# eflynn8/pharmacophore-diffusion

Hardware: AMD Instinct MI355X
Metric: denoising steps/sec (batch x T) at 256-atom pocket, 6 centers (higher is better)
Workload: dtype f32; 1 GPU; BASELINE config 2: 256-atom pocket, 6 centers, T=500 schedule, batch=32 per GPU, dev.yml network; batch_per_gpu=32, n_prot=256, n_pharm=6, T=500, parallelism=graphs sharded over 1 GPU(s), no data-path collective

## Files before the change

### include/pfdyn.h

```cpp
#ifndef PFDYN_H
#define PFDYN_H

#include <stdint.h>

#ifdef __cplusplus
extern "C" {
#endif

#define PF_ABI_VERSION 1

typedef struct pf_handle pf_handle;
typedef void* pf_stream;

typedef enum pf_status {
    PF_OK = 0,
    PF_ERR_ARG = -1,
    PF_ERR_HIP = -2,
    PF_ERR_STATE = -3,
    PF_ERR_WEIGHT = -4,
    PF_ERR_EXCHANGE = -5
} pf_status;

#define PF_NORM_MEAN 0
#define PF_NORM_VALUE 1
// ... 40 lines not shown
                        const float* dev_prot_x, const float* dev_prot_h,
                        int64_t n_pp, const int32_t* host_pp_src, const int32_t* host_pp_dst, pf_stream stream);

int pf_set_pocket_batch_host(pf_handle* h, int32_t B, const int32_t* host_prot_ptr, const int32_t* host_pharm_ptr,
                             const float* host_prot_x, const float* host_prot_h,
                             int64_t n_pp, const int32_t* host_pp_src, const int32_t* host_pp_dst, pf_stream stream);

int pf_set_pocket_groups(pf_handle* h, int32_t B, const int32_t* host_rep);

int pf_declare_onehot_features(pf_handle* h, int32_t is_onehot);

int64_t pf_build_pp_edges(pf_handle* h, int32_t B, const int32_t* host_prot_ptr, const float* dev_prot_x,
                          int32_t max_num_neighbors, int32_t* host_src, int32_t* host_dst, int64_t capacity,
                          pf_stream stream);

int pf_dynamics_forward(pf_handle* h, const float* dev_prot_x, const float* dev_pharm_x, const float* dev_pharm_h,
                        const float* dev_t , float* dev_eps_h , float* dev_eps_x ,
                        pf_stream stream);

int pf_sample_begin(pf_handle* h, const float* dev_init_pharm_com ,
                    const float* dev_noise0 , pf_stream stream);
int pf_denoise_step(pf_handle* h, const pf_step_coef* coef, const float* dev_noise ,
                    int32_t endpoint_param_coord, int32_t endpoint_param_feat, pf_stream stream);
int pf_sample_end(pf_handle* h, float feat_norm_constant, float* dev_x0 , float* dev_h0 ,
                  pf_stream stream);
int pf_sample_status(pf_handle* h, int32_t* n_timeouts);
int pf_sample_frame(pf_handle* h, float feat_norm_constant, float* dev_x , float* dev_h ,
                    pf_stream stream);
int pf_prepare_timesteps(pf_handle* h, const float* host_t, int32_t n, pf_stream stream);
int pf_sample(pf_handle* h, int32_t n_steps, const pf_step_coef* host_coef, const float* dev_noise,
              const float* dev_init_pharm_com, int32_t endpoint_param_coord, int32_t endpoint_param_feat,
              float feat_norm_constant, float* dev_x0, float* dev_h0, float* dev_traj_x, float* dev_traj_h,
              pf_stream stream);

int pf_param_count(pf_handle* h, int64_t* n_params, int32_t* n_tensors);
int pf_param_layout(pf_handle* h, int32_t index, const char** name, int64_t* offset, int64_t* numel);
int pf_train_forward(pf_handle* h, const float* dev_prot_x , const float* dev_pharm_x ,
                     const float* dev_pharm_h , const float* dev_t , float dropout_p, uint32_t seed,
                     float* dev_eps_h, float* dev_eps_x, pf_stream stream);
int pf_train_backward(pf_handle* h, const float* dev_g_eps_h , const float* dev_g_eps_x ,
                      float* dev_grad , pf_stream stream);
int pf_train_loss_forward(pf_handle* h, const float* dev_pharm_x0 , const float* dev_pharm_h0 ,
                          const int32_t* dev_t_int , const float* dev_eps_x , const float* dev_eps_h ,
                          const float* dev_alpha , const float* dev_sigma, int32_t n_timesteps, float feat_norm,
                          int32_t remove_com, int32_t weighted_loss, float dropout_p, uint32_t seed, float* dev_out ,
                          pf_stream stream);
int pf_train_loss_forward_ep(pf_handle* h, const float* dev_pharm_x0 , const float* dev_pharm_h0 ,
                             const int32_t* dev_t_int , const float* dev_eps_x , const float* dev_eps_h ,
                             const float* dev_alpha , const float* dev_sigma, int32_t n_timesteps, float feat_norm,
                             int32_t remove_com, int32_t weighted_loss, int32_t endpoint_param_coord, int32_t endpoint_param_feat,
                             float dropout_p, uint32_t seed, float* dev_out , pf_stream stream);
int pf_train_loss_backward(pf_handle* h, const float* dev_g_pos , const float* dev_g_feat ,
                           float* dev_grad , pf_stream stream);
int pf_train_loss_backward_out(pf_handle* h, const float* dev_g_out , float* dev_grad , pf_stream stream);
int pf_set_flat_params(pf_handle* h, const float* dev_flat , pf_stream stream);
int pf_get_flat_params(pf_handle* h, float* dev_flat , pf_stream stream);
int pf_adam_step(pf_handle* h, float* dev_params, const float* dev_grad, float* dev_exp_avg, float* dev_exp_avg_sq,
                 int64_t step, float lr, float beta1, float beta2, float eps, float weight_decay, pf_stream stream);
#define PF_TRAIN_F32 0
#define PF_TRAIN_BF16 1
int pf_train_set_precision(pf_handle* h, int32_t precision);
int pf_train_get_precision(pf_handle* h, int32_t* precision);
int pf_debug_set_dropout_masks(pf_handle* h, const float* dev_masks);
int pf_debug_dropout_mask(pf_handle* h, int32_t layer, int32_t which, float dropout_p, uint32_t seed,
                          float* dev_out , pf_stream stream);

int64_t pf_debug_get_edges(pf_handle* h, int32_t etype, int32_t* host_src, int32_t* host_dst, int64_t capacity,
                           pf_stream stream);
int pf_debug_conv_layer(pf_handle* h, int32_t layer, const float* dev_prot_x, const float* dev_pharm_x,
                        const float* dev_h_prot , const float* dev_v_prot ,
                        const float* dev_h_pharm, const float* dev_v_pharm,
                        float* dev_out_h_prot, float* dev_out_v_prot, float* dev_out_h_pharm, float* dev_out_v_pharm,
                        pf_stream stream);
#define PF_NUM_KERNEL_CLASSES 9
int pf_profile_enable(pf_handle* h, uint32_t kernel_mask);
int pf_profile_read(pf_handle* h, double* total_ms , int64_t* launches , pf_stream stream);
int pf_profile_read_train(pf_handle* h, double* total_ms , int64_t* launches , pf_stream stream);
int pf_debug_work(pf_handle* h, double* flops, double* bytes, int64_t* n_edges , double* executed_flops,
                  int64_t* executed_edges , pf_stream stream);
int pf_debug_counts(pf_handle* h, int64_t* out , pf_stream stream);
int pf_debug_kernel_family(pf_handle* h, int32_t layer, int32_t* rows_per_wave);
int pf_debug_ahead(pf_handle* h, int64_t* out , pf_stream stream);
int pf_debug_pa_check(pf_handle* h, int64_t* violations , pf_stream stream);
int pf_debug_xchg_timeouts(pf_handle* h, int32_t* n);
int pf_debug_xchg_fault(pf_handle* h, int32_t drop_word, int32_t poll_max);
int pf_debug_last_eps(pf_handle* h, float* dev_eps_h , float* dev_eps_x , pf_stream stream);
int pf_debug_l0_hoist(pf_handle* h, int32_t* rows_per_wave);
int pf_debug_chain(pf_handle* h, int32_t kind, int32_t layer, int32_t sub, int32_t n_rows, const float* dev_s_in,
                   const float* dev_v_in, float* dev_s_out, float* dev_v_out, pf_stream stream);

#ifdef __cplusplus
}
#endif
#endif
```

### pharmacophore-diffusion_amd/_lib.py

```python
import ctypes
import os

_HERE = os.path.dirname(os.path.abspath(__file__))
LIB_PATH = os.environ.get("PFDYN_LIB") or os.path.join(_HERE, "csrc", "libpfdyn.so")

PF_ABI_VERSION = 1
PF_NORM_MEAN, PF_NORM_VALUE, PF_NORM_GRAPH = 0, 1, 2


class PfConfig(ctypes.Structure):
    _fields_ = [
        ("abi_version", ctypes.c_int32), ("pharm_nf", ctypes.c_int32), ("rec_nf", ctypes.c_int32),
        ("vector_size", ctypes.c_int32), ("n_hidden_scalars", ctypes.c_int32), ("n_convs", ctypes.c_int32),
        ("n_message_gvps", ctypes.c_int32), ("n_update_gvps", ctypes.c_int32), ("n_noise_gvps", ctypes.c_int32),
        ("message_norm_mode", ctypes.c_int32), ("message_norm_value", ctypes.c_float),
        ("ff_k", ctypes.c_int32), ("pf_k", ctypes.c_int32),
        ("cutoff_pp", ctypes.c_float), ("cutoff_pf", ctypes.c_float), ("cutoff_fp", ctypes.c_float),
        ("cutoff_ff", ctypes.c_float), ("rbf_dmax", ctypes.c_float), ("rbf_dim", ctypes.c_int32),
    ]


class PfStepCoef(ctypes.Structure):
    _fields_ = [("t", ctypes.c_float), ("alpha_t_given_s", ctypes.c_float), ("var_terms", ctypes.c_float),
                ("sigma", ctypes.c_float), ("ep_zt", ctypes.c_float), ("ep_pred", ctypes.c_float)]


_P, _I32, _I64, _F = ctypes.c_void_p, ctypes.c_int32, ctypes.c_int64, ctypes.c_float
SYMBOLS = {
    "pf_version": (ctypes.c_char_p, []),
    "pf_last_error": (ctypes.c_char_p, [_P]),
    "pf_create": (ctypes.c_int, [ctypes.POINTER(PfConfig), ctypes.POINTER(_P)]),
    "pf_destroy": (None, [_P]),
    "pf_set_weight": (ctypes.c_int, [_P, ctypes.c_char_p, _P, _I32, ctypes.POINTER(_I64)]),
    "pf_commit_weights": (ctypes.c_int, [_P]),
    "pf_set_pocket_batch": (ctypes.c_int, [_P, _I32, _P, _P, _P, _P, _I64, _P, _P, _P]),
    "pf_set_pocket_batch_host": (ctypes.c_int, [_P, _I32, _P, _P, _P, _P, _I64, _P, _P, _P]),
    "pf_set_pocket_groups": (ctypes.c_int, [_P, _I32, _P]),
    "pf_declare_onehot_features": (ctypes.c_int, [_P, _I32]),
    "pf_build_pp_edges": (_I64, [_P, _I32, _P, _P, _I32, _P, _P, _I64, _P]),
    "pf_dynamics_forward": (ctypes.c_int, [_P, _P, _P, _P, _P, _P, _P, _P]),
    "pf_sample_begin": (ctypes.c_int, [_P, _P, _P, _P]),
    "pf_denoise_step": (ctypes.c_int, [_P, ctypes.POINTER(PfStepCoef), _P, _I32, _I32, _P]),
    "pf_sample_end": (ctypes.c_int, [_P, _F, _P, _P, _P]),
    "pf_sample_status": (ctypes.c_int, [_P, ctypes.POINTER(ctypes.c_int32)]),
    "pf_prepare_timesteps": (ctypes.c_int, [_P, _P, _I32, _P]),
    "pf_sample_frame": (ctypes.c_int, [_P, _F, _P, _P, _P]),
    "pf_sample": (ctypes.c_int, [_P, _I32, ctypes.POINTER(PfStepCoef), _P, _P, _I32, _I32, _F, _P, _P, _P, _P, _P]),
    "pf_param_count": (ctypes.c_int, [_P, ctypes.POINTER(_I64), ctypes.POINTER(_I32)]),
    "pf_param_layout": (ctypes.c_int, [_P, _I32, ctypes.POINTER(ctypes.c_char_p), ctypes.POINTER(_I64), ctypes.POINTER(_I64)]),
    "pf_train_forward": (ctypes.c_int, [_P, _P, _P, _P, _P, _F, ctypes.c_uint32, _P, _P, _P]),
    "pf_train_backward": (ctypes.c_int, [_P, _P, _P, _P, _P]),
    "pf_train_loss_forward": (ctypes.c_int, [_P, _P, _P, _P, _P, _P, _P, _P, ctypes.c_int32, ctypes.c_float, ctypes.c_int32,
                                             ctypes.c_int32, ctypes.c_float, ctypes.c_uint32, _P, _P]),
    "pf_train_loss_forward_ep": (ctypes.c_int, [_P, _P, _P, _P, _P, _P, _P, _P, ctypes.c_int32, ctypes.c_float, ctypes.c_int32,
                                                ctypes.c_int32, ctypes.c_int32, ctypes.c_int32, ctypes.c_float, ctypes.c_uint32, _P, _P]),
    "pf_train_loss_backward": (ctypes.c_int, [_P, _P, _P, _P, _P]),
    "pf_train_loss_backward_out": (ctypes.c_int, [_P, _P, _P, _P]),
    "pf_set_flat_params": (ctypes.c_int, [_P, _P, _P]),
    "pf_get_flat_params": (ctypes.c_int, [_P, _P, _P]),
    "pf_adam_step": (ctypes.c_int, [_P, _P, _P, _P, _P, _I64, _F, _F, _F, _F, _F, _P]),
    "pf_train_set_precision": (ctypes.c_int, [_P, _I32]),
    "pf_train_get_precision": (ctypes.c_int, [_P, ctypes.POINTER(_I32)]),
    "pf_debug_set_dropout_masks": (ctypes.c_int, [_P, _P]),
    "pf_debug_dropout_mask": (ctypes.c_int, [_P, _I32, _I32, _F, ctypes.c_uint32, _P, _P]),
    "pf_debug_get_edges": (_I64, [_P, _I32, _P, _P, _I64, _P]),
    "pf_debug_conv_layer": (ctypes.c_int, [_P, _I32] + [_P] * 11),
    "pf_profile_enable": (ctypes.c_int, [_P, ctypes.c_uint32]),
    "pf_profile_read": (ctypes.c_int, [_P, ctypes.POINTER(ctypes.c_double), ctypes.POINTER(_I64), _P]),
    "pf_profile_read_train": (ctypes.c_int, [_P, ctypes.POINTER(ctypes.c_double), ctypes.POINTER(_I64), _P]),
    "pf_debug_work": (ctypes.c_int, [_P, ctypes.POINTER(ctypes.c_double), ctypes.POINTER(ctypes.c_double),
                                     ctypes.POINTER(_I64), ctypes.POINTER(ctypes.c_double), ctypes.POINTER(_I64), _P]),
    "pf_debug_counts": (ctypes.c_int, [_P, ctypes.POINTER(_I64), _P]),
    "pf_debug_kernel_family": (ctypes.c_int, [_P, ctypes.c_int32, ctypes.POINTER(ctypes.c_int32)]),
    "pf_debug_last_eps": (ctypes.c_int, [_P, _P, _P, _P]),
    "pf_debug_xchg_timeouts": (ctypes.c_int, [_P, ctypes.POINTER(ctypes.c_int32)]),
    "pf_debug_xchg_fault": (ctypes.c_int, [_P, _I32, _I32]),
    "pf_debug_ahead": (ctypes.c_int, [_P, ctypes.POINTER(_I64), _P]),
    "pf_debug_pa_check": (ctypes.c_int, [_P, ctypes.POINTER(_I64), _P]),
    "pf_debug_l0_hoist": (ctypes.c_int, [_P, ctypes.POINTER(ctypes.c_int32)]),
    "pf_debug_chain": (ctypes.c_int, [_P, _I32, _I32, _I32, _I32, _P, _P, _P, _P, _P]),
}

_lib = None


def load():
    global _lib
    if _lib is not None:
        return _lib
    if not os.path.exists(LIB_PATH):
        raise ImportError(
            f"{LIB_PATH} is missing: the HIP extension has not been built "
            "(run `python -c 'import __graft_entry__ as g; g.build()'` or `make -C pharmacophore-diffusion_amd/csrc`). "
            "There is no CPU fallback.")
    lib = ctypes.CDLL(LIB_PATH)
    for name, (res, args) in SYMBOLS.items():
        fn = getattr(lib, name)
        fn.restype = res
        fn.argtypes = args
    _lib = lib
    return lib


class PfError(RuntimeError):
    pass


def check(lib, handle, rc, what):
    if rc < 0:
        msg = lib.pf_last_error(handle)
        raise PfError(f"{what} failed ({rc}): {msg.decode() if msg else ''}")
    return rc
```

### pharmacophore-diffusion_amd/csrc/pf_device.h

```cpp
#pragma once
#include <stdint.h>

#define PF_S 128
#define PF_V 16
#define PF_R 16
#define PF_MAXF 64
#define PF_MAXK 16
#define PF_MAX_GVPS 8

enum { ET_FF = 0, ET_PF = 1, ET_FP = 2, ET_PP = 3 };

#if defined(__HIP_DEVICE_COMPILE__)
#define PF_AS1 __attribute__((address_space(1)))
#else
#define PF_AS1
#endif
typedef const float PF_AS1* pf_gcf;

struct GvpW {
    pf_gcf a_wh;
    pf_gcf a_wu;
    pf_gcf a_main;
    pf_gcf a_main_c;
    pf_gcf a_gate_c;
// ... 103 lines not shown
    const int* esrc;
    const int* edst;
    const float4* xn;
    const float* h;
    const float* v;
    float* msg_s;
    float* msg_v;
    const GvpW* w;
    const float* pre;
    int n_gvps;
    float rbf_mu[PF_R];
    float rbf_inv_sigma;
    float* sv_z; float* sv_g; float* sv_v; size_t sv_stride;
    int bf16;
    pf_gcf rg[4];
    const int* reg; int nreg, regB, ngroups4, ngroups8;
    pf_gcf rgs[4]; int rgs_stride;
    const float* zs;
    const float* ptab;
    int ptab_gstride;
    const int* ptype;
    const int* eorig;
    const int* l0_gid;
    const float* l0c;
    int ngroups_sel;
    const int* need; int need_stamp;
    int pa_abs;
    pf_gcf n16[4]; int n16_stride[4];
    int uni_base[3], uni_s01, uni_s2g, uni_pa_groups;
    int ptab16_off[4];
    const float* pcen; int pcen_nf;
    const float* x0_static;
    const int* pa_skip;
    int* cnt_snap;
    int* pa_gstamp; int pa_serial;
};

#define L0H_WR 0
#define L0H_WSH 2048
#define L0H_B 4224
#define L0H_WH0 4352
#define L0H_WU 4384
#define L0H_BG 4672
#define L0H_WHT 4736
#define L0H_WHT_PF 21120
#define L0H_B_PF 37504
#define L0H_SIZE (37504 + 128)
#define L0C_WHT_FF 0
#define L0C_B_FF 16384
#define L0C_WHT_FP 16512
#define L0C_B_FP 32896
#define L0C_SIZE (32896 + 128)
#define L0_NTAB 4
struct L0HoistParams {
    const float* src;
    float* l0c;
    const int* esrc; const int* edst; const float4* xn; int Epp;
    float rbf_mu0, rbf_mu_step, rbf_inv_sigma;
    float* zs;
    const float* enc_w; const float* enc_b; const float* enc_lw; const float* enc_lb;
    int rec_nf, nt;
    const float* t_dev;
    float t_host[64];
    float* ptab;
    const float* prot_h0; int Np; int* ptype; int* flag;
};

struct NodeW {
    pf_gcf ln1_w; pf_gcf ln1_b;
    pf_gcf ln2_w; pf_gcf ln2_b;
    const GvpW PF_AS1* upd;
};

struct UnitParams {
    const float* s_in; const float* v_in; float* s_out; float* v_out;
    int n, kind, n_gvps, pharm_nf;
    const float* stream;
    int skip_gvps;
    const float* ln_w; const float* ln_b;
    float* sv_z; float* sv_g; float* sv_v; size_t sv_stride;
    int n16_stride;
};

struct NodeParams {
    const NodeTile* tiles;
    int ntiles;
    const int* in_start;
    const int* in_cnt;
    int N;
    int pp_slot;
    const int* row_ids;
    const int* dyn_cnt;
    const float* msg_s;
    const float* msg_v;
    int zero_row;
    const float* h_in; const float* v_in;
    float* h_out; float* v_out;
    const int* gid;
    const float* gnorm;
    int B;
    int norm_mode; float norm_value;
    NodeW w[2];
    int n_upd;
    uint32_t drop_thr; float drop_scale; uint32_t seed; int layer;
    const float* mask_override;
    int xcd_n;
    int st_n0, st_n;
    int grp;
    int grp_pa;
    pf_gcf rg_upd[2];
    pf_gcf rgs_upd[2]; int rgs_stride[2];
    float* sv_z; float* sv_g; float* sv_v; size_t sv_stride;
};

struct ZeroList {
    void* p[8];
    unsigned long long nbytes[8];
    int cnt;
};
struct FusedParams {
    const int* in_start; const int* in_cnt; int N, pp_slot;
    const float* msg_s; const float* msg_v; int zero_row, grp, grp_pa;
    const int* gid; const float* gnorm; int B, norm_mode; float norm_value;
    pf_gcf ln1_w[2], ln1_b[2], ln2_w[2], ln2_b[2];
    int n_upd;
    pf_gcf chain[4]; int chain_stride[4];
    pf_gcf upd_pharm; int upd_pharm_stride;
    const float* htab; int htab_gstride;
    const int* ptype;
    float* h_out; float* v_out;
    const int* pharm_ptr; int Np, n_edge_items;
    int xcd_split, nff_cap, npf_cap;
    int uni_ff_base, uni_pf_base, uni_strides, uni_groups;
    const int4* rec;
    const float* hcen;
};

struct TailParams {
    const int* in_start; const int* in_cnt; int N;
    const float* msg_s; const float* msg_v; int zero_row, grp;
    const float* h_in; const float* v_in;
    const int* gid; const float* gnorm; int B, norm_mode; float norm_value;
    pf_gcf ln1_w, ln1_b, ln2_w, ln2_b;
    int n_upd, n_head;
    pf_gcf chain; int chain_stride;
    int pharm_nf;
    float* eps_h; float* eps_x;
};

struct HeadParams {
    const NodeTile* tiles;
    int ntiles;
    int node_base;
    const float* h; const float* v;
    const GvpW* gvps;
    int n_gvps;
    const float* a_out;
    const float* b_out;
    int pharm_nf;
    float* eps_h;
    float* eps_x;
    unsigned int* xchg;
    int xchg_fault;
    unsigned int* xchg2;
};
#define PF_XCHG_STRIDE 20
#define PF_XCHG_EMPTY 0xffffffffu
#ifdef __HIPCC__
__device__ __forceinline__ unsigned int pf_xchg_word(const float v) {
    const unsigned int b = __float_as_uint(v);
    return b == PF_XCHG_EMPTY ? 0x7fc00000u : b;
}
#endif

struct CenHoistParams {
    int on, Nf, nf;
    float t_next;
    const float* pharm_h;
    const float* noise;
    float a_ts, var, sigma, ep_zt, ep_pred; int ep_feat;
    const float* enc_w; const float* enc_b; const float* enc_lw; const float* enc_lb;
    const float* blk;
    float* cen_h; float* cen_p;
    unsigned int* xchg2;
};

struct EncodeParams {
    int Np, Nf;
    const float* prot_h0;
    const float* pharm_h;
    const float* t;
    float t_scalar;
    const int* gid;
    int rec_nf, pharm_nf;
    const float* w[2]; const float* b[2]; const float* ln_w[2]; const float* ln_b[2];
    float* h_out;
};

struct BuildParams {
    int B, Np_tot;
    const int* prot_ptr; const int* pharm_ptr;
    const float4* xn;
    const int* reg;
    int* dyn_cnt;
    int* act_ids;
    const int* reg_act;
    int* esrc; int* edst;
    int* eorig;
    int* in_start; int* in_cnt; int N;
    int ff_k, pf_k;
    float r2_ff, r2_pf;
    float* gnorm;
    const int* pp_cnt;
    const int* pa_static;
    const int* rep_base;
    int* need; int need_stamp;
    const int* pfq_cnt;
    int norm_mode;
// ... 86 lines not shown
```

### pharmacophore-diffusion_amd/csrc/pf_host.cpp

```cpp
#include <hip/hip_runtime.h>

#include <algorithm>
#include <cmath>
#include <cstdio>
#include <cstdlib>
#include <cstring>
#include <ctime>
#include <map>
#include <string>
#include <unordered_map>
#include <climits>
#include <vector>

#include "../../include/pfdyn.h"
#include "pf_device.h"
#include "pf_train.h"

#define L0_PTAB_SLOTS 2048

extern "C" {
void pfk_edge_msg(const EdgeParams* p, int layer0, hipStream_t s);
void pfk_edge_msg_coop(const EdgeParams* p, int layer0, hipStream_t s);
void pfk_edge_msg_coop2(const EdgeParams* p, int layer0, hipStream_t s);
void pfk_node_update_coop(const NodeParams* p, int layer0, hipStream_t s);
void pfk_node_head_coop(const NodeParams* p, const HeadParams* hp, int layer0, hipStream_t s);
void pfk_noise_head_coop(const HeadParams* p, hipStream_t s);
void pfk_node_update(const NodeParams* p, int layer0, hipStream_t s);
void pfk_noise_head(const HeadParams* p, hipStream_t s);
void pfk_rg_edge(const EdgeParams* p, const EncodeParams* enc, int layer0, int rg, int split, int rgp, hipStream_t s);
void pfk_l0_hoist(const L0HoistParams* p, int what, hipStream_t s);
void pfk_rg_node(const NodeParams* p, const HeadParams* hp, const EncodeParams* enc, int layer0, int rg, int split, hipStream_t s);
void pfk_rg_unit(const UnitParams* p, hipStream_t s);
void pfk_rg_node_hs_build(const NodeParams* p, const HeadParams* hp, const StepParams* sp, const BuildParams* bp, int* xstat, int poll_sleep,
                          int avoid, int poll_max, const CenHoistParams* cp, const EdgeParams* es, const EncodeParams* ees, int spec_groups,
                          hipStream_t s);
void pfk_n16_edge(const EdgeParams* p, const EncodeParams* enc, int layer0, hipStream_t s);
void pfk_pa_spec(const EdgeParams* es, const EncodeParams* ees, int groups, int after, int k, int frac, int* word, hipStream_t s);
void pfk_pa_check(const int* dyn_cnt, const int* cnt_snap, const int* reg, const int* pa_same, const int* gstamp, int serial, int B,
                  unsigned long long* out, hipStream_t s);
void pfk_n16_unit(const UnitParams* p, hipStream_t s);
void pfk_n16_fused(const EdgeParams* p, const FusedParams* f, const EncodeParams* enc, hipStream_t s);
void pfk_n16_tail(const TailParams* t, const StepParams* sp, const BuildParams* bp, hipStream_t s);
void pfk_rg_tail(const NodeParams* p, const HeadParams* hp, const StepParams* sp, const BuildParams* bp, hipStream_t s);
void pfk_encode(const EncodeParams* p, hipStream_t s);
void pfk_encode_build(const EncodeParams* e, const BuildParams* b, hipStream_t s);
void pfk_encode_build_pre(const EncodeParams* e, const BuildParams* b, const PreParams* pp, hipStream_t s);
void pfk_build_edges(const BuildParams* p, hipStream_t s);
void pfk_load_coords(const float* src, float4* xn, int n, const int* gid, const float* shift, float sign, hipStream_t s);
void pfk_load_noise0(const float* nz, float4* xn, float* hf, int n, int nf, hipStream_t s);
void pfk_copy(const float* src, float* dst, size_t n, hipStream_t s);
void pfk_zero_multi(const ZeroList* z, hipStream_t s);
void pfk_copy2(const float* a, float* da, size_t na, const float* b, float* db, size_t nb, hipStream_t s);
void pfk_verify_copies(const float* x0, const float* h0, const int* gid, const int* prot_ptr, const int* rep_base, int Np, int rec_nf,
                       int* flag, hipStream_t s);
void pfk_scale_copy(const float* src, float* dst, size_t n, float sc, hipStream_t s);
void pfk_segment_mean(const float4* xn, const int* ptr, int base, int B, float* out, hipStream_t s);
void pfk_step_update(const StepParams* p, hipStream_t s);
void pfk_step_build(const StepParams* sp, const BuildParams* bp, int fast, hipStream_t s);
void pfk_export_coords(const float4* xn, int base, int n, const int* gid, const float* add, const float* sub,
                       float* out, hipStream_t s);
void pfk_bwd_head(const BwdHeadParams* p, int nblocks, hipStream_t s);
void pfk_bwd_node(const BwdNodeParams* p, int nblocks, hipStream_t s);
void pfk_bwd_edge_level(const BwdEdgeLevelParams* p, int nblocks, hipStream_t s);
void pfk_fix_apply(long long* A, float* G, size_t n, const float* fix, hipStream_t s);
void pfk_fix_apply_rows(const NodeTile* tiles, int ntiles, const int* dyn_cnt, const int* row_ids, long long* A_h, float* G_h,
                        long long* A_v, float* G_v, const float* fix, hipStream_t s);
void pfk_fix_scale(const float* g_h, int n_h, const float* g_x, int n_x, float* fix, hipStream_t s);
void pfk_bwd_encode(const BwdEncodeParams* p, int nblocks, hipStream_t s);
void pfk_enc_group(const float* G_h, const int* prot_ptr, const int* ptype, int B, int rec_nf, float* Gg, hipStream_t s);
void pfk_fix_enc_group(long long* A_h, float* G_h, const float* fix, const int* prot_ptr, const int* ptype, int B, int rec_nf, float* Gg,
                       int Np, int Nf, const int* onehot_flag, hipStream_t s);
void pfk_train_reduce(const ReduceParams* p, hipStream_t s);
void pfk_gather_weights(const float* flat, const int* map, size_t n, float* packed, hipStream_t s);
void pfk_n16_split_words(const float* flat, const int4* tab, size_t n, float* packed, hipStream_t s);
void pfk_pack_gvp(const float* W, const GvpT* g, int n_gvps, float* out_b, float* out_f, const ScaleArgs* sa, hipStream_t s);
void pfk_loss_prepare(const LossParams* p, hipStream_t s);
void pfk_loss_eval(const LossParams* p, int ep_coord, int ep_feat, hipStream_t s);
void pfk_scale_loss(float* gx, int nx, const float* a, const float* a2, float* gh, int nh, const float* b, const float* b2, hipStream_t s);
void pfk_compact_node_rows(const NodeTile* tiles, int ntiles, const int* dyn_cnt, const int* row_ids, int N, int* list, int cap, int* ucnt,
                           hipStream_t s);
void pfk_compact_rows(const EdgeTile* tiles, const int* et_tile0, int n_et, const int* dyn_cnt, int* rlist, int* ccnt, hipStream_t s);
void pfk_adam(float* p, const float* g, float* m, float* v, size_t n, float lr, float b1, float b2, float eps, float wd,
              float bc1, float bc2_sqrt, float* mirror, hipStream_t s);
void pfk_drop_masks(const TrainCommon* c, uint32_t stream, int n_elems, float* out, hipStream_t s);
void pfk_pp_radius(const float4* xn, const int* prot_ptr, int B, float r2, int maxn, int* deg, const int* row_off,
                   int* src, int* dst, int pass, hipStream_t s);
void pfk_wide_encode(const WideEncParams* p, hipStream_t s);
void pfk_wide_edge(const WideEdgeParams* p, hipStream_t s);
void pfk_wide_node(const WideNodeParams* p, hipStream_t s);
}

namespace {

static std::string g_create_error;

struct RawTensor {
    std::vector<int64_t> shape;
    std::vector<float> data;
};

static const char* kEtKey[4] = {"pharm_ff_pharm", "prot_pf_pharm", "pharm_fp_prot", "prot_pp_prot"};
static const char* kNtKey[2] = {"prot", "pharm"};

inline int rho(int r, int hl) { return (r & 3) + 8 * (r >> 2) + 4 * hl; }

static void linspace_f32(float start, float end, int steps, float* out) {
    const float step = (end - start) / (float)(steps - 1);
    const int half = steps / 2;
    for (int i = 0; i < steps; ++i) out[i] = i < half ? start + step * (float)i : end - step * (float)(steps - i - 1);
}

}

struct LaunchPolicy {
    static constexpr int kCUs = 256, kSIMDs = 4 * kCUs;
    int n16_mask = 7;
    int tail_graphs_max = 256;
    int xcd_split = 1;
// ... 63 lines not shown
    std::vector<GvpW> h_gvp;
    int msg_base(int layer, int et) const { return ((layer * 4 + et) * cfg.n_message_gvps); }
    int upd_base(int layer, int nt) const { return n_msg_tot + (layer * 2 + nt) * cfg.n_update_gvps; }
    int head_base() const { return n_msg_tot + n_upd_tot; }
    int n_msg_tot = 0, n_upd_tot = 0;
    size_t enc_w[2]{}, enc_b[2]{}, enc_lw[2]{}, enc_lb[2]{};
    std::vector<size_t> ln_off;
    size_t out_a = 0, out_b = 0;
    size_t enc_a = 0, enc_bf = 0;
    bool use_pre = true;

    bool have_batch = false;
    int B = 0, Np = 0, Nf = 0, N = 0;
    int64_t Epp = 0, Ecap = 0;
    std::vector<int> h_prot_ptr, h_pharm_ptr;
    std::vector<int> h_reg;
    std::vector<int> h_cap;
    int n_edge_tiles = 0, n_node_tiles = 0, n_head_tiles = 0;
    int zero_row = 0;
    int n_edge_tiles_last = 0, n_node_tiles_last = 0;
    bool prune = true;
    int n_edge_tiles_act = 0, n_node_tiles_act = 0;
    EdgeTile* d_edge_tiles_act = nullptr;
    NodeTile* d_node_tiles_act = nullptr;
    int *d_act_ids = nullptr, *d_reg_act = nullptr;
    void* d_ws = nullptr;
    size_t ws_capacity = 0;
    void* stage[2] = {nullptr, nullptr};
    size_t stage_cap[2] = {0, 0};
    hipEvent_t stage_ev[2] = {nullptr, nullptr};
    int stage_next = 0;
    void* d_tab[2] = {nullptr, nullptr};
    size_t tab_cap[2] = {0, 0};
    hipEvent_t tab_guard[2] = {nullptr, nullptr}, tab_up[2] = {nullptr, nullptr};
    bool tab_guard_set[2] = {false, false};
    int tab_next = 0;
    hipStream_t s_copy = nullptr;
    hipStream_t s_side = nullptr;
    int l0_state = 0;
    int* l0flag_host = nullptr;
    hipEvent_t l0flag_ev = nullptr;
    size_t tws_capacity = 0;
    int *d_prot_ptr = nullptr, *d_pharm_ptr = nullptr, *d_gid = nullptr, *d_reg = nullptr, *d_dyn_cnt = nullptr,
        *d_esrc = nullptr, *d_edst = nullptr, *d_in_start = nullptr, *d_in_cnt = nullptr, *d_pp_cnt = nullptr;
    EdgeTile* d_edge_tiles = nullptr;
    NodeTile* d_node_tiles = nullptr;
    NodeTile* d_head_tiles = nullptr;
    float4* d_xn = nullptr;
    float *d_prot_x0 = nullptr, *d_prot_h0 = nullptr, *d_pharm_h = nullptr, *d_t = nullptr, *d_h[2] = {nullptr, nullptr},
          *d_v[2] = {nullptr, nullptr}, *d_msg_s = nullptr, *d_msg_v = nullptr, *d_eps_h = nullptr, *d_eps_x = nullptr,
          *d_com_init = nullptr, *d_com_tmp = nullptr, *d_gnorm = nullptr, *d_pre = nullptr;
    int* d_pfq_cnt = nullptr;
    std::vector<int> pending_rep;
    bool share_ok = false;
    int share_check = 1;
    int* d_reg_share = nullptr;
    int* d_pa_static = nullptr;
    int* d_rep_base = nullptr;
    int* d_need = nullptr;
    int need_stamp = 0, edges_stamp = 0;
    long share_rows = 0;
    std::vector<int> h_share_start, h_share_cnt;
    bool share_disable = false;
    bool train_rg_node = true;
    bool train_rg_edge = true;
    bool train_rg_head = true;
    float *t_hsv_z = nullptr, *t_hsv_g = nullptr, *t_hsv_v = nullptr;
    bool t_head_saved = false;
    unsigned int* d_xchg = nullptr;
    int* d_xstat = nullptr;
    int* xstat_host = nullptr;
    int xstat_ack = 0;
    int xchg_fault = 0, xchg_poll_max = 0;
    size_t n16_l0h[4] = {0, 0, 0, 0}, n16_l0h_stride[4] = {0, 0, 0, 0};
    size_t l0c_off = 0;
    bool cen_hoist = true;
    float *d_cen_h = nullptr, *d_cen_p = nullptr, *d_snap[2] = {nullptr, nullptr};
    unsigned int* d_xchg2 = nullptr;
    int snap_cur = -1;
    std::vector<float> t_plan; size_t plan_pos = 0;
    bool cen_valid = false; float cen_t = 0.f; uint64_t cen_wver = 0;
    bool last_cen = false;
    bool pa_spec = true;
    bool spec_valid = false; float spec_t = 0.f; uint64_t spec_wver = 0;
    int step_id = 2;
    int *d_pa_stamp = nullptr, *d_pa_same = nullptr;
    bool e0_saved = false; EdgeParams e0{}; EncodeParams ep0{}; int e0_groups = 0;
    int last_spec = 0;
    int* d_pa_cnt = nullptr;
    int pa_spec_split = 0;
    bool pa_check = false;
    int pa_serial = 0, spec_serial = 0;
    int* d_pa_gstamp = nullptr;
    unsigned long long* d_pa_chk = nullptr;
    bool no_fixed_shapes = false;
    ScaleArgs pend_scale{}; bool has_pend_scale = false;
    bool no_fix_fuse = false;
    bool train_bf16 = false;
    bool train_node_save = true;
    std::vector<float*> t_nsv_z, t_nsv_g, t_nsv_v;
    std::vector<char> t_node_saved;
    std::vector<int> t_grp;
    bool sampling = false;
    int max_np = 0, max_nf = 0;
    bool edges_built = false;
    bool edges_share = false;
    std::vector<size_t> rg_msg, rg_upd;
    std::vector<size_t> rgs_msg, rgs_upd, rgs_upd_stride;
    size_t rgs_msg_stride = 0;
    std::vector<size_t> n16_msg, n16_upd;
    size_t n16_msg_stride = 0, n16_upd_stride = 0;
    size_t n16_begin = 0;
    bool n16_stale = false;
    bool split_record = false;
    std::vector<int4> split_pending, split_tab;
    int4* d_split_tab = nullptr; size_t n_split_tab = 0;
    size_t n16_l0[4] = {0, 0, 0, 0}, n16_l0_stride[4] = {0, 0, 0, 0};
    size_t n16_fused[2] = {0, 0}, n16_fused_stride[2] = {0, 0};
    size_t n16_tail = 0, n16_tail_stride = 0;
    bool tail_done = false;
    int last_tail = 0;
    float *d_msg_s2 = nullptr, *d_msg_v2 = nullptr;
    std::vector<int> last_family;
    int last_hoist = 0;
    bool l0_hoist = true;
    size_t l0h_off = 0;
    uint64_t w_version = 1, zs_version = 0, ptab_version = 0;
    bool l0_onehot = false;
    bool coords_custom = false;
    bool zs_batch_coords = false;
    float* d_l0c = nullptr;
    float* d_ptab = nullptr;
    std::unordered_map<uint32_t, int> ptab_slot;
    int *d_eorig = nullptr, *d_ptype = nullptr, *d_l0flag = nullptr;
    int4* d_rec = nullptr; bool rec_valid = false;
    float *d_zs = nullptr, *d_ptab_pg = nullptr;
    bool enc_on_the_fly = true;
    bool step_build_fast = true;
    bool rg_compact = true;
    bool fuse_head = true;
    void init_tuning() {
        if (const char* e = getenv("PFDYN_NO_PRE")) use_pre = atoi(e) == 0;
        if (const char* e = getenv("PFDYN_NO_FUSE_HEAD")) fuse_head = atoi(e) == 0;
        if (const char* e = getenv("PFDYN_NO_PRUNE")) prune = atoi(e) == 0;
        if (const char* e = getenv("PFDYN_NO_ENC_FLY")) enc_on_the_fly = atoi(e) == 0;
        if (const char* e = getenv("PFDYN_NO_COMPACT")) rg_compact = atoi(e) == 0;
        if (const char* e = getenv("PFDYN_NO_FAST_BUILD")) step_build_fast = atoi(e) == 0;
        if (const char* e = getenv("PFDYN_NO_L0_HOIST")) l0_hoist = atoi(e) == 0;
        if (const char* e = getenv("PFDYN_NO_CENTER_HOIST")) cen_hoist = atoi(e) == 0;
        if (const char* e = getenv("PFDYN_NO_PA_SPEC")) pa_spec = atoi(e) == 0;
        if (const char* e = getenv("PFDYN_PA_SPEC_SPLIT")) pa_spec_split = !strcmp(e, "mid") ? -1 : (!strcmp(e, "step") ? -2 : std::max(atoi(e), 0));
        if (const char* e = getenv("PFDYN_PA_CHECK")) pa_check = atoi(e) != 0;
        if (const char* e = getenv("PFDYN_NO_POCKET_SHARE")) share_disable = atoi(e) != 0;
        if (const char* e = getenv("PFDYN_TRAIN_TILE_NODE")) train_rg_node = atoi(e) == 0;
        if (const char* e = getenv("PFDYN_TRAIN_TILE_EDGE")) train_rg_edge = atoi(e) == 0;
        if (const char* e = getenv("PFDYN_TRAIN_TILE_HEAD")) train_rg_head = atoi(e) == 0;
        if (const char* e = getenv("PFDYN_TRAIN_NODE_RECOMPUTE")) train_node_save = atoi(e) == 0;
        if (const char* e = getenv("PFDYN_TRAIN_BF16")) train_bf16 = atoi(e) != 0;
        if (const char* e = getenv("PFDYN_NO_FIX_FUSE")) no_fix_fuse = atoi(e) != 0;
        if (const char* e = getenv("PFDYN_NO_FIXED_SHAPES")) no_fixed_shapes = atoi(e) != 0;
        pol.from_env();
    }

    float* d_flat = nullptr;
    size_t nparams = 0;
    std::vector<std::pair<std::string, std::pair<size_t, size_t>>> flat_layout;
    GvpT* d_gvpt = nullptr;
    std::vector<int> h_map;
    int* d_map = nullptr;
    size_t n_packed = 0;
    void* d_tws = nullptr;
    std::vector<float*> t_H, t_V, t_msg_s, t_msg_v;
    std::vector<float*> t_sv_z, t_sv_g, t_sv_v;
    float *t_gs_buf = nullptr, *t_gv_buf = nullptr;
    int et_tile0[5] = {0, 0, 0, 0, 0};
    int et_tile0_act[5] = {0, 0, 0, 0, 0};
    float *t_G_h[2] = {nullptr, nullptr}, *t_G_v[2] = {nullptr, nullptr}, *t_gagg_s = nullptr, *t_gagg_v = nullptr,
          *t_gpart = nullptr, *t_geps_h = nullptr, *t_geps_x = nullptr;
    long long *t_A_h = nullptr, *t_A_v = nullptr;
    float* d_lpart = nullptr;
    void* d_tA = nullptr;
    size_t tA_capacity = 0;
    bool tA_dirty = false;
    int enc_begin = 0, enc_n = 0;
    float* t_gpart_enc = nullptr;
    TensorSeg* d_tseg = nullptr; int n_tseg = 0;
    int n_gvpt = 0;
    float* d_wpack = nullptr;
    uint64_t wpack_version = ~0ull;
    float *t_lx0c = nullptr, *t_lag = nullptr, *t_lsg = nullptr, *t_lcom2 = nullptr, *t_lgx = nullptr, *t_lgh = nullptr, *t_lout = nullptr;
    bool t_have_loss = false;
    float* t_Gg = nullptr;
    int* t_ulist = nullptr;
    int t_ucap = 0;
    size_t t_clist_cap = 0, t_ulist_cap = 0;
    hipEvent_t cmp_ev[3] = {nullptr, nullptr, nullptr};
    int *t_clist = nullptr, *t_ccnt = nullptr;
    float* t_fix = nullptr;
    int t_nblk = 0;
    const float* t_mask_override = nullptr;
    bool t_have_fwd = false;
    bool t_ws_ready = false;
    TrainCommon t_common{};
    mutable std::unordered_map<std::string, size_t> flat_index;
    mutable bool flat_index_ok = false;
    size_t flat_offset(const std::string& name) const {
        if (!flat_index_ok) {
            flat_index.clear();
            for (const auto& kv : flat_layout) flat_index.emplace(kv.first, kv.second.first);
            flat_index_ok = true;
        }
        const auto it = flat_index.find(name);
        return it == flat_index.end() ? (size_t)-1 : it->second;
    }
    std::vector<int> edge_fx;

    enum { K_ENCODE = 0, K_BUILD, K_EDGE, K_NODE, K_HEAD, K_STEP, K_EDGE_COOP, K_NODE_COOP, K_EDGE_LAST,
           K_BWD_HEAD, K_BWD_NODE, K_BWD_EDGE_LEVEL, K_BWD_REST, K_NUM };
    unsigned prof_mask = 0;
    std::vector<std::pair<hipEvent_t, hipEvent_t>> prof_ev[K_NUM];
    size_t prof_used[K_NUM] = {};
};

namespace {

#define PF_FAIL(h, code, ...)                                   \
    do {                                                        \
        char _b[512];                                           \
        snprintf(_b, sizeof(_b), __VA_ARGS__);                  \
        (h)->err = _b;                                          \
        return (code);                                          \
    } while (0)

// ... 766 lines not shown
        e.x0_static = h->d_prot_x0;
        if (dc.spec_have && pa_ahead_ok(h, e, shared)) { e.pa_skip = h->d_pa_same; h->last_spec = 1; }
    }
    if (l == 0 && dc.cen_have && h->n16_l0h[ET_FF] != 0) {
        for (int et : {(int)ET_FF, (int)ET_FP}) { e.n16[et] = h->d_w + h->n16_l0h[et]; e.n16_stride[et] = (int)h->n16_l0h_stride[et]; }
        e.pcen = h->d_cen_p; e.pcen_nf = h->Nf; h->last_cen = true;
    }
    e.ngroups_sel = region_groups(h, shared, 0, e.nreg, 16);
    int stride[3], cap[3], grp[3] = {0, 0, 0};
    bool uni = l == 0 && h->pol.fused_uni && !shared && e.reg == h->d_reg && e.nreg == 4 * h->B && h->B <= 64 && !e.pa_abs && !e.need &&
               uniform_regions(h, 3, stride, cap);
    for (int et = 0; et < 3 && uni; ++et) { grp[et] = (cap[et] + 15) / 16; uni = grp[et] > 0 && grp[et] < 8; }
    if (uni) {
        for (int et = 0; et < 3; ++et) e.uni_base[et] = h->h_reg[(size_t)et * h->B];
        e.uni_s01 = stride[0] | (stride[1] << 16);
        e.uni_s2g = stride[2] | (grp[0] << 16) | (grp[1] << 19) | (grp[2] << 22) | ((h->B - 1) << 25);
        e.uni_pa_groups = region_groups(h, shared, 3 * h->B, 4 * h->B, 16);
    }
    dc.rg = 4;
    if (l == 0 && e.x0_static && pa_ahead_ok(h, e, shared)) {
        e.cnt_snap = h->d_pa_cnt;
        h->e0 = e; h->ep0 = dc.ep; h->e0_saved = true;
        h->e0_groups = region_groups(h, shared, 3 * h->B, 4 * h->B, 16);
    }
}
static void edge_launch(DynCall& dc, int l) {
    pf_handle* h = dc.h; hipStream_t s = dc.s; const pf_config& c = h->cfg; const bool train = dc.train;
    const bool last = dc.last = (l == c.n_convs - 1), pruned = dc.pruned = (l == prune_layer(h));
    EdgeParams& e = dc.e; int &rg = dc.rg, &rgp = dc.rgp;
    e = edge_params_base(h, l, last, pruned);
    e.h = train ? h->t_H[l] : h->d_h[dc.cur]; e.v = train ? h->t_V[l] : h->d_v[dc.cur];
    e.msg_s = train ? h->t_msg_s[l] : h->d_msg_s; e.msg_v = train ? h->t_msg_v[l] : h->d_msg_v;
    if (dc.fuse_l0node && l == 1) { e.msg_s = h->d_msg_s2; e.msg_v = h->d_msg_v2; }
    e.pre = (l == 0 && dc.pre_ready) ? h->d_pre : nullptr;
    if (train) { e.sv_z = h->t_sv_z[l]; e.sv_g = h->t_sv_g[l]; e.sv_v = h->t_sv_v[l]; e.sv_stride = (size_t)std::max<int64_t>(h->Ecap, 1); }
    const bool shared = dc.shared = dc.share && pruned && l == 0;
    if ((last || pruned) && h->rg_compact && (last ? 2 : 4) * h->B <= 1024) {
        e.reg = shared ? h->d_reg_share : h->d_reg; e.regB = h->B; e.nreg = (last ? 2 : 4) * h->B; e.pa_abs = shared ? 1 : 0;
        if (shared) { e.need = h->d_need; e.need_stamp = h->edges_stamp; }
        e.ngroups4 = region_groups(h, shared, 0, e.nreg, 4); e.ngroups8 = region_groups(h, shared, 0, e.nreg, 8);
    }
    if (train && h->train_bf16) e.bf16 = 1;
    rg = train ? ((h->train_rg_edge && h->train_rg_node && !h->train_bf16) ? h->pol.rg_mode(e.ntiles) : 0)
               : h->pol.rg_mode(shared ? (int)((h->share_rows + 31) / 32) : e.ntiles);
    rgp = 0;
    if (dc.hoist && l == 0 && rg) {
        e.zs = h->d_zs; e.ptab = dc.l0_ptab; e.ptab_gstride = dc.l0_gstride; e.ptype = h->d_ptype; e.eorig = h->d_eorig; e.l0_gid = h->d_gid; e.l0c = h->d_l0c;
        rgp = rg;
        if (e.nreg > 0 && pruned) {
            rg = shared ? ((h->share_rows >= h->pol.rg2_rows_min || (long)e.ntiles * 32 >= h->pol.rg2_rows_min_hoist) ? 2 : 1)
                        : ((long)e.ntiles * 32 >= h->pol.rg2_rows_min_hoist ? 2 : 1);
            const int rgp_pol = shared ? rg : ((long)e.ntiles * 32 >= h->pol.rg2p_rows_min ? 2 : 1);
            if (h->pol.l0_rga) rg = h->pol.l0_rga;
            rgp = h->pol.l0_rgp ? h->pol.l0_rgp : std::max(rg, rgp_pol);
            if (rg == 2) rgp = 2;
            e.ngroups_sel = region_groups(h, shared, 0, 3 * h->B, 4 * rg) + region_groups(h, shared, 3 * h->B, e.nreg, 4 * rgp);
        }
        h->last_hoist = 4 * rgp;
    }
    const bool n16e = !train && rg && dc.n16_batch && (l > 0 ? (h->pol.n16_mask & 1) != 0 : dc.n16_l0);
    if (n16e) edge_n16_form(dc, l);
    h->last_family.resize(c.n_convs);
    h->last_family[l] = rg ? 4 * rg : ((!train && e.ntiles <= ((last || pruned) ? std::max(h->pol.coop_edge_max, h->pol.coop2_edge_max) : std::max(h->pol.coop_edge_max, h->pol.coop2_dense_max))) ? 128 : 32);
    for (int et = 0; et < 4; ++et) { e.rgs[et] = h->d_w + h->rgs_msg[(size_t)l * 4 + et]; e.rgs_stride = (int)h->rgs_msg_stride; }
    const int esplit = (rg == 1 && e.ntiles * 8 <= h->pol.rg_split_max && !e.zs) ? 1 : 0;
    const int pc = edge_prof_class(last, c.n_convs);
    if (n16e && dc.fuse_l0node && l == 1) {
        FusedParams& fz = dc.fz;
        fz.chain[ET_FF] = h->d_w + h->n16_fused[0]; fz.chain_stride[ET_FF] = (int)h->n16_fused_stride[0];
        fz.chain[ET_PF] = h->d_w + h->n16_fused[1]; fz.chain_stride[ET_PF] = (int)h->n16_fused_stride[1];
        fz.upd_pharm = h->d_w + h->n16_upd[(size_t)0 * 2 + 1]; fz.upd_pharm_stride = (int)h->n16_upd_stride;
        fz.htab = dc.l0_ptab + (size_t)3 * c.rec_nf * PF_S; fz.htab_gstride = dc.l0_gstride; fz.ptype = h->d_ptype; fz.hcen = h->last_cen ? h->d_cen_h : nullptr;
        fz.h_out = h->d_h[dc.cur]; fz.v_out = h->d_v[dc.cur];
        fz.pharm_ptr = h->d_pharm_ptr; fz.Np = h->Np; fz.n_edge_items = e.ngroups_sel;
        fz.nff_cap = region_groups(h, shared, 0, std::min(h->B, e.nreg), 16); fz.npf_cap = region_groups(h, shared, h->B, e.nreg, 16);
        fz.xcd_split = ((h->pol.xcd_split & 1) && 2 * h->B <= 64 && h->max_nf <= 16) ? 1 : 0;
        int stride[2], cap[2];
        bool uni = fz.xcd_split && h->pol.fused_uni && e.reg == h->d_reg && e.nreg == 2 * h->B && uniform_regions(h, 2, stride, cap);
        for (int et = 0; et < 2 && uni; ++et) uni = cap[et] > 0 && (cap[et] + 15) / 16 < 256;
        if (uni) {
            fz.uni_ff_base = h->h_reg[0]; fz.uni_pf_base = h->h_reg[(size_t)h->B];
            fz.uni_strides = stride[0] | (stride[1] << 16); fz.uni_groups = ((cap[0] + 15) / 16) | (((cap[1] + 15) / 16) << 8);
        }
        h->last_family[l] = 17;
        { ProfScope ps(h, pf_handle::K_EDGE_LAST, s); pfk_n16_fused(&e, &fz, &dc.ep, s); }
    }
    else if (n16e) {
        if (l == 0 && e.pa_skip && h->d_pa_gstamp && h->d_pa_chk)
            pfk_pa_check(h->d_dyn_cnt, h->d_pa_cnt, e.reg, e.pa_skip, h->d_pa_gstamp, h->spec_serial, h->B, h->d_pa_chk, s);
        ProfScope ps(h, pc, s); pfk_n16_edge(&e, &dc.ep, l == 0, s);
    }
    else if (rg) { ProfScope ps(h, pc, s); pfk_rg_edge(&e, dc.enc_fly ? &dc.ep : nullptr, l == 0, rg, esplit, rgp, s); }
    else if (e.ntiles <= h->pol.coop_edge_max && !train) { ProfScope ps(h, pc, s); pfk_edge_msg_coop(&e, l == 0, s); }
    else if (e.ntiles <= ((last || pruned) ? h->pol.coop2_edge_max : h->pol.coop2_dense_max) && !train) { ProfScope ps(h, pc, s); pfk_edge_msg_coop2(&e, l == 0, s); }
    else { ProfScope ps(h, pf_handle::K_EDGE, s); pfk_edge_msg(&e, l == 0, s); }
}
static void fused_take_node(DynCall& dc, const NodeParams& n) {
    pf_handle* h = dc.h; FusedParams& fz = dc.fz;
    fz.in_start = n.in_start; fz.in_cnt = n.in_cnt; fz.N = n.N; fz.pp_slot = n.pp_slot;
    fz.rec = (h->rec_valid && h->d_rec && n.pp_slot == 2 && !dc.shared) ? h->d_rec : nullptr;
    fz.msg_s = n.msg_s; fz.msg_v = n.msg_v; fz.zero_row = n.zero_row; fz.grp = n.grp; fz.grp_pa = n.grp_pa;
    fz.gid = n.gid; fz.gnorm = n.gnorm; fz.B = n.B; fz.norm_mode = n.norm_mode; fz.norm_value = n.norm_value; fz.n_upd = n.n_upd;
    for (int nt = 0; nt < 2; ++nt) { fz.ln1_w[nt] = n.w[nt].ln1_w; fz.ln1_b[nt] = n.w[nt].ln1_b; fz.ln2_w[nt] = n.w[nt].ln2_w; fz.ln2_b[nt] = n.w[nt].ln2_b; }
}
static void node_save_levels(pf_handle* h, int l, NodeParams& n) {
    n.sv_z = h->t_nsv_z[l]; n.sv_g = h->t_nsv_g[l]; n.sv_v = h->t_nsv_v[l]; n.sv_stride = (size_t)2 * h->N;
    h->t_node_saved[l] = 1;
}
static void tail_launch(DynCall& dc, const NodeParams& n, int form) {
    pf_handle* h = dc.h; hipStream_t s = dc.s; const pf_config& c = h->cfg;
    const HeadParams hp = head_params(h, dc.eps_h, dc.eps_x); TailParams tp{};
    if (form == 16) {
        tp.in_start = n.in_start; tp.in_cnt = n.in_cnt; tp.N = n.N; tp.h_in = n.h_in; tp.v_in = n.v_in;
        tp.msg_s = n.msg_s; tp.msg_v = n.msg_v; tp.zero_row = n.zero_row; tp.grp = n.grp;
        tp.gid = n.gid; tp.gnorm = n.gnorm; tp.B = n.B; tp.norm_mode = n.norm_mode; tp.norm_value = n.norm_value;
        tp.ln1_w = n.w[1].ln1_w; tp.ln1_b = n.w[1].ln1_b; tp.ln2_w = n.w[1].ln2_w; tp.ln2_b = n.w[1].ln2_b;
        tp.n_upd = n.n_upd; tp.n_head = c.n_noise_gvps; tp.chain = h->d_w + h->n16_tail; tp.chain_stride = (int)h->n16_tail_stride;
        tp.pharm_nf = c.pharm_nf; tp.eps_h = dc.eps_h; tp.eps_x = dc.eps_x;
    }
    const bool sn = share_next(h);
    const BuildParams bpn = build_params(h, sn);
    { ProfScope ps(h, pf_handle::K_HEAD, s); if (form == 16) pfk_n16_tail(&tp, dc.step, &bpn, s); else pfk_rg_tail(&n, &hp, dc.step, &bpn, s); }
    build_done(h, sn);
    h->tail_done = true; h->last_tail = form; dc.head_done = true;
}
static float cen_hoist_plan(DynCall& dc) {
    pf_handle* h = dc.h;
    if (!(h->cen_hoist && dc.t_scalar && !h->t_plan.empty() && h->last_hoist == 16 && h->l0c_off != 0 && h->n16_l0h[ET_FF] != 0 &&
          h->snap_cur >= 0 && dc.step->h_snap_out != nullptr && h->d_xchg2 && dc.fuse_l0node)) return NAN;
    return planned_next_t(h, *dc.t_scalar, &h->plan_pos);
}
static void cen_hoist_params(DynCall& dc, float t_next, CenHoistParams& cp, HeadParams& hp) {
    pf_handle* h = dc.h; const StepParams* step = dc.step;
    cp.on = 1; cp.Nf = h->Nf; cp.nf = h->cfg.pharm_nf; cp.t_next = t_next; cp.pharm_h = h->d_snap[h->snap_cur]; cp.noise = step->noise;
    cp.a_ts = step->a_ts; cp.var = step->var; cp.sigma = step->sigma; cp.ep_zt = step->ep_zt; cp.ep_pred = step->ep_pred; cp.ep_feat = step->ep_feat;
    cp.enc_w = h->d_w + h->enc_w[1]; cp.enc_b = h->d_w + h->enc_b[1]; cp.enc_lw = h->d_w + h->enc_lw[1]; cp.enc_lb = h->d_w + h->enc_lb[1];
    cp.blk = h->d_w + h->l0c_off; cp.cen_h = h->d_cen_h; cp.cen_p = h->d_cen_p; cp.xchg2 = hp.xchg2 = h->d_xchg2;
    h->cen_valid = true; h->cen_t = t_next; h->cen_wver = h->w_version;
}
static int pa_ahead_plan(DynCall& dc, EdgeParams& es, EncodeParams& ees) {
    pf_handle* h = dc.h; const pf_config& c = h->cfg;
    if (!(h->e0_saved && h->pa_spec && !h->t_plan.empty() && dc.t_scalar && h->d_pa_stamp && !share_next(h))) return 0;
    float tn = planned_next_t(h, *dc.t_scalar, nullptr);
    if (tn != tn) return 0;
    l0_prepare_t(h, &tn, 1, dc.s);
    uint32_t bits; memcpy(&bits, &tn, 4);
    es = h->e0; es.pa_skip = nullptr; es.pcen = nullptr;
    es.ptab = h->d_ptab + (size_t)h->ptab_slot[bits] * L0_NTAB * c.rec_nf * PF_S;
    for (int et = 0; et < 4; ++et) { es.n16[et] = h->d_w + h->n16_l0[et]; es.n16_stride[et] = (int)h->n16_l0_stride[et]; }
    ees = h->ep0; ees.t_scalar = tn;
    h->spec_valid = true; h->spec_t = tn; h->spec_wver = h->w_version;
    es.pa_serial = h->spec_serial = ++h->pa_serial; es.pa_gstamp = h->d_pa_gstamp;
    return h->e0_groups;
}
static void merged_step_launch(DynCall& dc, const NodeParams& n, HeadParams& hp) {
    pf_handle* h = dc.h; hipStream_t s = dc.s; const pf_config& c = h->cfg;
    hp.xchg = h->d_xchg; hp.xchg_fault = h->xchg_fault;
    CenHoistParams cp{}; EdgeParams es{}; EncodeParams ees{};
    const float t_next = cen_hoist_plan(dc);
    const int spec_groups = pa_ahead_plan(dc, es, ees);
    if (t_next == t_next) cen_hoist_params(dc, t_next, cp, hp);
    const bool sn = share_next(h);
    BuildParams bpn = build_params(h, sn);
    const bool with_rec = h->d_rec && !sn && c.ff_k == 0 && bpn.act_ids && !bpn.pa_static && h->last_hoist == 16 && dc.fuse_l0node;
    if (with_rec) { bpn.rec = h->d_rec; bpn.ptype = h->d_ptype; }
    const bool split = spec_groups > 0 && h->pa_spec_split != 0;
    if (split) {
        const int frac = h->pa_spec_split == -1 ? 128 : (h->pa_spec_split == -2 ? (int)((((uint32_t)h->pa_serial * 2654435761u) >> 16) & 255) + 1 : 0);
        pfk_pa_spec(&es, &ees, spec_groups, 0, std::max(h->pa_spec_split, 0), frac, h->d_pa_cnt + h->B, s);
    }
    { ProfScope ps(h, pf_handle::K_HEAD, s); pfk_rg_node_hs_build(&n, &hp, dc.step, &bpn, h->d_xstat, h->pol.xchg_sleep, h->pol.hsb_avoid, h->xchg_poll_max, &cp, &es, &ees, split ? 0 : spec_groups, s); }
    if (split) pfk_pa_spec(&es, &ees, spec_groups, 1, 0, 0, h->d_pa_cnt + h->B, s);
    build_done(h, sn, with_rec);
    h->tail_done = true; h->last_tail = 2;
}
static void node_launch(DynCall& dc, int l) {
    pf_handle* h = dc.h; hipStream_t s = dc.s; const pf_config& c = h->cfg; const bool train = dc.train;
    NodeParams n = node_params_base(h, l, dc.last, dc.pruned);
    if (dc.shared) n.pp_slot = 3;
    n.msg_s = dc.e.msg_s; n.msg_v = dc.e.msg_v; n.h_in = dc.e.h; n.v_in = dc.e.v;
    n.h_out = train ? h->t_H[l + 1] : h->d_h[dc.cur ^ 1]; n.v_out = train ? h->t_V[l + 1] : h->d_v[dc.cur ^ 1];
    if (train) { n.drop_thr = h->t_common.drop_thr; n.drop_scale = h->t_common.drop_scale; n.seed = h->t_common.seed; n.layer = l; n.mask_override = h->t_common.mask_override; }
    n.grp = dc.rg ? 4 * dc.rg : 32; n.grp_pa = dc.rgp ? 4 * dc.rgp : n.grp;
    if (train) { h->t_grp.resize(c.n_convs); h->t_grp[l] = n.grp; h->t_node_saved.resize(c.n_convs); h->t_node_saved[l] = 0; }
    for (int nt = 0; nt < 2; ++nt) { n.rgs_upd[nt] = h->d_w + h->rgs_upd[(size_t)l * 2 + nt]; n.rgs_stride[nt] = (int)h->rgs_upd_stride[(size_t)l * 2 + nt]; }
    const EncodeParams* enc = dc.enc_fly ? &dc.ep : nullptr;
    if (dc.fuse_l0node && l == 0) fused_take_node(dc, n);
    else if (dc.rg) {
        const int rgn = (long)n.ntiles * 32 >= h->pol.rg2_rows_min_node ? 2 : 1;
        const bool fuse = dc.last && !train && h->fuse_head && h->n_head_tiles == n.ntiles;
        const int nsplit = (!train && rgn == 1 && n.ntiles * 8 <= (fuse ? h->pol.rg_split_max_head : h->pol.rg_split_max_node)) ? 1 : 0;
        const bool tail = fuse && dc.step != nullptr && l > 0 && (h->pol.n16_mask & 8) && h->B <= h->pol.tail_graphs_max && dc.enc_fly && step_build_fast_ok(h);
        if (tail) tail_launch(dc, n, (h->pol.tail_form == 16 && h->n16_tail != 0) ? 16 : 4);
        else if (fuse) {
            if (nsplit && h->pol.node_xcds > 0 && n.ntiles * 8 <= 32 * h->pol.node_xcds) n.xcd_n = h->pol.node_xcds;
            if (nsplit && l > 0 && h->pol.node_static) { n.st_n0 = h->Np; n.st_n = h->Nf; }
            HeadParams hp = head_params(h, dc.eps_h, dc.eps_x);
            const bool hsb = n.st_n > 0 && dc.step != nullptr && h->pol.hs_build && dc.enc_fly && step_build_fast_ok(h) &&
                             h->B <= 256 && !(h->prof_mask & (1u << pf_handle::K_STEP)) && h->d_xchg && h->d_xstat;
            if (hsb) merged_step_launch(dc, n, hp);
            else { ProfScope ps(h, pf_handle::K_HEAD, s); pfk_rg_node(&n, &hp, enc, l == 0, rgn, nsplit, s); }
            dc.head_done = true;
        } else {
            if (train && h->train_node_save) node_save_levels(h, l, n);
            ProfScope ps(h, pf_handle::K_NODE_COOP, s); pfk_rg_node(&n, nullptr, enc, l == 0, rgn, nsplit, s);
        }
    }
    else if (dc.last && !train && h->fuse_head && n.ntiles <= h->pol.coop_node_max && h->n_head_tiles == n.ntiles) {
        const HeadParams hp = head_params(h, dc.eps_h, dc.eps_x);
        { ProfScope ps(h, pf_handle::K_HEAD, s); pfk_node_head_coop(&n, &hp, l == 0, s); }
        dc.head_done = true;
    }
    else if (train && h->train_rg_node && h->pol.rg_mode(n.ntiles) > 0) {
        n.grp = 32; n.grp_pa = 32;
        if (h->train_node_save) node_save_levels(h, l, n);
        ProfScope ps(h, pf_handle::K_NODE_COOP, s); pfk_rg_node(&n, nullptr, nullptr, l == 0, h->pol.rg_mode(n.ntiles), 0, s);
    }
    else if (n.ntiles <= h->pol.coop_node_max && !train) { ProfScope ps(h, pf_handle::K_NODE_COOP, s); pfk_node_update_coop(&n, l == 0, s); }
    else { ProfScope ps(h, pf_handle::K_NODE, s); pfk_node_update(&n, l == 0, s); }
}
static void head_launch(DynCall& dc) {
    pf_handle* h = dc.h; hipStream_t s = dc.s; const pf_config& c = h->cfg; const bool train = dc.train;
    HeadParams hp = head_params(h, dc.eps_h, dc.eps_x);
    hp.h = train ? h->t_H[c.n_convs] : h->d_h[dc.cur]; hp.v = train ? h->t_V[c.n_convs] : h->d_v[dc.cur];
    if (train) h->t_head_saved = false;
    if (!dc.head_done && train && h->train_rg_head && !h->rg_msg.empty() && h->Nf > 0) {
        UnitParams up{};
        up.s_in = hp.h + (size_t)h->Np * PF_S; up.v_in = hp.v + (size_t)h->Np * 48; up.s_out = dc.eps_h; up.v_out = dc.eps_x;
        up.n = h->Nf; up.kind = 3; up.n_gvps = c.n_noise_gvps; up.pharm_nf = c.pharm_nf;
        up.stream = h->d_w + h->rg_upd[(size_t)(c.n_convs - 1) * 2 + 1]; up.skip_gvps = c.n_update_gvps;
        up.sv_z = h->t_hsv_z; up.sv_g = h->t_hsv_g; up.sv_v = h->t_hsv_v; up.sv_stride = (size_t)h->Nf;
        { ProfScope ps(h, pf_handle::K_HEAD, s); pfk_rg_unit(&up, s); }
        h->t_head_saved = true; dc.head_done = true;
    }
    if (!dc.head_done) { ProfScope ps(h, pf_handle::K_HEAD, s); if (hp.ntiles <= h->pol.coop_node_max) pfk_noise_head_coop(&hp, s); else pfk_noise_head(&hp, s); }
}
static int run_dynamics(pf_handle* h, float* eps_h, float* eps_x, hipStream_t s, const float* t_scalar = nullptr, bool train = false, const StepParams* step = nullptr) {
    if (h->wide && !train) return run_dynamics_wide(h, eps_h, eps_x, s, t_scalar);
    const pf_config& c = h->cfg;
    h->tail_done = false; h->last_tail = 0;
    DynCall dc{};
    dc.h = h; dc.s = s; dc.eps_h = eps_h; dc.eps_x = eps_x; dc.t_scalar = t_scalar; dc.train = train; dc.step = step;
    dc.cen_have = !train && h->cen_valid && h->edges_built && t_scalar != nullptr && *t_scalar == h->cen_t && h->cen_wver == h->w_version;
    h->cen_valid = false; h->last_cen = false;
    dc.spec_have = !train && h->spec_valid && h->edges_built && t_scalar != nullptr && *t_scalar == h->spec_t && h->spec_wver == h->w_version;
    h->spec_valid = false; h->last_spec = 0; h->e0_saved = false;
    if (!train) n16_refresh(h, s);
    dc.ep = encode_params(h, t_scalar, train ? h->t_H[0] : h->d_h[0]);
    if (const int rc = dyn_prologue(dc)) return rc;
    dyn_hoist_prepare(dc);
    h->last_hoist = 0;
    dc.fuse_l0node = !train && dc.n16_batch && (long)h->n_edge_tiles_act * 32 <= h->pol.n16_fuse_rows_max && (h->pol.n16_mask & 4) && (h->pol.n16_mask & 1) && dc.hoist && c.n_convs == 2 && prune_layer(h) == 0 && c.pf_k > 0 &&
                     c.n_update_gvps >= 1 && h->rg_compact && 2 * h->B <= 1024 && h->d_msg_s2 != nullptr && h->n16_fused[0] != 0;
    for (int l = 0; l < c.n_convs; ++l, dc.cur ^= 1) { edge_launch(dc, l); node_launch(dc, l); }
    head_launch(dc);
    h->edges_built = h->tail_done;
    hipError_t e = hipGetLastError();
    if (e != hipSuccess) PF_FAIL(h, PF_ERR_HIP, "kernel launch failed: %s", hipGetErrorString(e));
    return PF_OK;
}

struct ZeroBatch {
    ZeroList z{};
    hipStream_t s;
    explicit ZeroBatch(hipStream_t st) : s(st) {}
    void add(void* p, size_t nbytes) {
        if (!p || nbytes == 0) return;
        if (z.cnt == 8) flush();
        z.p[z.cnt] = p; z.nbytes[z.cnt] = nbytes; ++z.cnt;
    }
    void flush() { pfk_zero_multi(&z, s); z.cnt = 0; }
};

static int check_ready(pf_handle* h, bool need_batch) {
    if (!h) return PF_ERR_ARG;
    if (!h->committed) PF_FAIL(h, PF_ERR_STATE, "weights not committed (pf_commit_weights)");
    if (need_batch && !h->have_batch) PF_FAIL(h, PF_ERR_STATE, "no pocket batch set (pf_set_pocket_batch)");
    return PF_OK;
}

}

extern "C" {

const char* pf_version(void) { return "libpfdyn 0.1 (gfx950, fp32 MFMA)"; }

const char* pf_last_error(const pf_handle* h) { return h ? h->err.c_str() : g_create_error.c_str(); }

int pf_create(const pf_config* cfg, pf_handle** out) {
    if (!cfg || !out) { g_create_error = "null argument"; return PF_ERR_ARG; }
    *out = nullptr;
    auto bad = [&](const char* m) { g_create_error = m; return PF_ERR_ARG; };
    if (cfg->abi_version != PF_ABI_VERSION) return bad("abi_version mismatch");
    if (cfg->vector_size != 16 && cfg->vector_size != PFW_MAXV) return bad("vector_size must be 16 or 32");
    if (cfg->n_hidden_scalars < 64 || cfg->n_hidden_scalars > PFW_MAXS || cfg->n_hidden_scalars % 32)
        return bad("n_hidden_scalars must be a multiple of 32 in 64..256");
    if (cfg->rbf_dim != PF_R) return bad("rbf_dim must be 16");
    if (cfg->pharm_nf < 1 || cfg->pharm_nf > 16 || cfg->rec_nf < 1) return bad("pharm_nf must be in 1..16, rec_nf >= 1");
    if (cfg->n_convs < 1 || cfg->n_message_gvps < 1 || cfg->n_message_gvps > PF_MAX_GVPS || cfg->n_update_gvps < 1 ||
        cfg->n_update_gvps > PF_MAX_GVPS || cfg->n_noise_gvps < 1 || cfg->n_noise_gvps > PF_MAX_GVPS)
        return bad("layer counts out of range");
    if (cfg->ff_k < 0 || cfg->ff_k > PF_MAXK || cfg->pf_k < 0 || cfg->pf_k > PF_MAXK) return bad("ff_k / pf_k must be in 0..16");
    if (cfg->message_norm_mode < 0 || cfg->message_norm_mode > 2) return bad("bad message_norm_mode");
    if (cfg->message_norm_mode == PF_NORM_VALUE && !(cfg->message_norm_value > 0)) return bad("message_norm_value must be > 0");
    int ndev = 0;
    if (hipGetDeviceCount(&ndev) != hipSuccess || ndev == 0) {
        g_create_error = "no HIP device available (libpfdyn has no CPU fallback)";
        return PF_ERR_HIP;
    }
    pf_handle* h = new pf_handle();
    h->cfg = *cfg;
    h->init_tuning();
    h->spec = cfg->n_hidden_scalars == PF_S && cfg->vector_size == PF_V;
    const char* wv = getenv("PFDYN_WIDE");
    h->wide = !h->spec || (wv && atoi(wv) != 0);
    if (h->wide) {
        h->l0_hoist = h->cen_hoist = h->pa_spec = false;
        h->pol.hs_build = 0; h->pol.n16_mask = 0;
    }
    *out = h;
    return PF_OK;
}

void pf_destroy(pf_handle* h) {
// ... 152 lines not shown
                for (int k = 0; k < 17; ++k) blk[L0H_WH0 + k] = wh[(size_t)0 * 17 + k];
                for (int k = 0; k < 17 * 16; ++k) blk[L0H_WU + k] = wu[k];
                for (int k = 0; k < 16; ++k) blk[L0H_BG + k] = h->raw[g.prefix + "scalar_to_vector_gates.bias"].data[k];
                const GvpSpec gp = msg_spec(c, 0, ET_PF, 0);
                const std::vector<float>& Wp = h->raw[gp.prefix + "to_feats_out.0.weight"].data;
                for (int f = 0; f < PF_S; ++f) {
                    for (int k = 0; k < PF_S; ++k) blk[L0H_WHT_PF + (size_t)k * PF_S + f] = Wp[(size_t)f * Kin + k];
                    blk[L0H_B_PF + f] = h->raw[gp.prefix + "to_feats_out.0.bias"].data[f];
                }
            }
            h->l0h_off = push(h->h_w, blk);
            h->l0c_off = 0;
            if (g.vi == 17 && g.so == PF_S && g.si == PF_S + PF_R && g.vo == 16) {
                std::vector<float> cb(L0C_SIZE, 0.f);
                const int Kin = g.si + 17;
                for (int k2 = 0; k2 < 2; ++k2) {
                    const GvpSpec gc = msg_spec(c, 0, k2 == 0 ? ET_FF : ET_FP, 0);
                    const std::vector<float>& Wc = h->raw[gc.prefix + "to_feats_out.0.weight"].data;
                    const std::vector<float>& bc = h->raw[gc.prefix + "to_feats_out.0.bias"].data;
                    const size_t wo = k2 == 0 ? L0C_WHT_FF : L0C_WHT_FP, bo = k2 == 0 ? L0C_B_FF : L0C_B_FP;
                    for (int f = 0; f < PF_S; ++f) {
                        for (int k = 0; k < PF_S; ++k) cb[wo + (size_t)k * PF_S + f] = Wc[(size_t)f * Kin + k];
                        cb[bo + f] = bc[f];
                    }
                }
                h->l0c_off = push(h->h_w, cb);
            }
        }
        if (h->spec) {
            h->rg_msg.assign((size_t)c.n_convs * 4, 0);
            h->rg_upd.assign((size_t)c.n_convs * 2, 0);
            std::vector<float> st;
            auto flush = [&]() { const size_t off = push(h->h_w, st); st.clear(); return off; };
            auto chain = [&](auto spec_of, int n, int half = -1) {
                GvpSpec prev;
                for (int j = 0; j < n; ++j) {
                    const GvpSpec g = spec_of(j);
                    pack_gvp_rg(h, g, j ? &prev : nullptr, st, half);
                    prev = g;
                }
                pack_flush_rg(h, prev, st);
            };
            for (int l = 0; l < c.n_convs; ++l)
                for (int et = 0; et < 4; ++et) {
                    chain([&](int j) { return msg_spec(c, l, et, j); }, c.n_message_gvps);
                    h->rg_msg[(size_t)l * 4 + et] = flush();
                }
            for (int l = 0; l < c.n_convs; ++l)
                for (int nt = 0; nt < 2; ++nt) {
                    if (l == c.n_convs - 1 && nt == 1) continue;
                    chain([&](int j) { return upd_spec(c, l, nt, j); }, c.n_update_gvps);
                    h->rg_upd[(size_t)l * 2 + nt] = flush();
                }
            chain([&](int j) { return upd_spec(c, c.n_convs - 1, 1, j); }, c.n_update_gvps);
            chain([&](int k) { return head_spec(c, k); }, c.n_noise_gvps);
            pack_out_rg(h, st);
            st.resize(st.size() + (size_t)RG_TAIL_PAD * 256, 0.f);
            h->rg_upd[(size_t)(c.n_convs - 1) * 2 + 1] = flush();
            h->rgs_msg.assign((size_t)c.n_convs * 4, 0);
            h->rgs_upd.assign((size_t)c.n_convs * 2, 0);
            h->rgs_upd_stride.assign((size_t)c.n_convs * 2, 0);
            for (int l = 0; l < c.n_convs; ++l)
                for (int et = 0; et < 4; ++et) {
                    for (int half = 0; half < 2; ++half) {
                        chain([&](int j) { return msg_spec(c, l, et, j); }, c.n_message_gvps, half);
                        if (half == 0) h->rgs_msg_stride = st.size();
                    }
                    h->rgs_msg[(size_t)l * 4 + et] = flush();
                }
            for (int l = 0; l < c.n_convs; ++l)
                for (int nt = 0; nt < 2; ++nt) {
                    const bool tail = l == c.n_convs - 1 && nt == 1;
                    for (int half = 0; half < 2; ++half) {
                        chain([&](int j) { return upd_spec(c, l, nt, j); }, c.n_update_gvps, half);
                        if (tail) {
                            chain([&](int k) { return head_spec(c, k); }, c.n_noise_gvps, half);
                            pack_out_rg(h, st);
                        }
                        if (half == 0) h->rgs_upd_stride[(size_t)l * 2 + nt] = st.size();
                    }
                    if (!tail) h->rgs_upd[(size_t)l * 2 + nt] = flush();
                }
            st.resize(st.size() + (size_t)RG_TAIL_PAD * 256, 0.f);
            h->rgs_upd[(size_t)(c.n_convs - 1) * 2 + 1] = flush();
        }
        h->n16_begin = h->spec ? h->h_w.size() : 0;
        if (h->spec && c.n_message_gvps >= 2 && c.n_update_gvps >= 1) {
            h->n16_msg.assign((size_t)c.n_convs * 4, 0);
            h->n16_upd.assign((size_t)c.n_convs * 2, 0);
            std::vector<float> st;
            auto chain16 = [&](auto spec_of, int n, int kind0, size_t& stride, int m0_at = -1) {
                for (int w = 0; w < 4; ++w) {
                    const size_t b0 = st.size();
                    for (int j = 0; j < n; ++j) pack_n16(h, spec_of(j), j == m0_at ? N16_M0F : (j == 0 ? kind0 : N16_GEN), w, st);
                    st.resize(st.size() + (size_t)N16_TAIL_PAD * 256, 0.f);
                    stride = st.size() - b0;
                }
                const size_t off = push(h->h_w, st);
                for (int4 r : h->split_pending) { r.x += (int)off; h->split_tab.push_back(r); }
                h->split_pending.clear();
                st.clear();
                return off;
            };
            for (int l = 0; l < c.n_convs; ++l)
                for (int et = 0; et < 4; ++et)
                    h->n16_msg[(size_t)l * 4 + et] = chain16([&](int j) { return msg_spec(c, l, et, j); }, c.n_message_gvps, N16_M0F, h->n16_msg_stride);
            for (int et = 0; et < 4; ++et)
                h->n16_l0[et] = chain16([&](int j) { return msg_spec(c, 0, et, j); }, c.n_message_gvps,
                                        (et == ET_PP || et == ET_PF) ? N16_M0H : N16_M0Z, h->n16_l0_stride[et]);
            for (int et = 0; et < 4; ++et)
                h->n16_l0h[et] = chain16([&](int j) { return msg_spec(c, 0, et, j); }, c.n_message_gvps, N16_M0H, h->n16_l0h_stride[et]);
            if (c.n_convs == 2)
                for (int k = 0; k < 2; ++k) {
                    const int et = k == 0 ? ET_FF : ET_PF, nt = k == 0 ? 1 : 0;
                    h->n16_fused[k] = chain16([&](int j) { return j < c.n_update_gvps ? upd_spec(c, 0, nt, j) : msg_spec(c, 1, et, j - c.n_update_gvps); },
                                              c.n_update_gvps + c.n_message_gvps, N16_GEN, h->n16_fused_stride[k], c.n_update_gvps);
                }
            for (int l = 0; l < c.n_convs; ++l)
                for (int nt = 0; nt < 2; ++nt)
                    h->n16_upd[(size_t)l * 2 + nt] = chain16([&](int j) { return upd_spec(c, l, nt, j); }, c.n_update_gvps, N16_GEN, h->n16_upd_stride);
            {
                const GvpSpec hl = head_spec(c, c.n_noise_gvps - 1);
                h->n16_tail = 0;
                if (c.pharm_nf <= 15 && c.n_noise_gvps >= 1 && hl.vi == 16 && hl.vo == 1 && hl.si == PF_S && hl.so == 64) {
                    for (int w = 0; w < 4; ++w) {
                        const size_t b0 = st.size();
                        for (int j = 0; j < c.n_update_gvps; ++j) pack_n16(h, upd_spec(c, c.n_convs - 1, 1, j), N16_GEN, w, st);
                        for (int k = 0; k + 1 < c.n_noise_gvps; ++k) pack_n16(h, head_spec(c, k), N16_GEN, w, st);
                        pack_n16_head_last(h, hl, w, st);
                        st.resize(st.size() + (size_t)N16_TAIL_PAD * 256, 0.f);
                        h->n16_tail_stride = st.size() - b0;
                    }
                    h->n16_tail = push(h->h_w, st);
                    for (int4 r : h->split_pending) { r.x += (int)h->n16_tail; h->split_tab.push_back(r); }
                    h->split_pending.clear();
                    st.clear();
                }
            }
        } else { h->n16_msg.clear(); h->n16_upd.clear(); h->n16_tail = 0; for (int et = 0; et < 4; ++et) h->n16_l0h[et] = 0; }
        while (h->h_w.size() % 64) h->h_w.push_back(0.f);
    };
    {
        std::map<std::string, RawTensor> keep;
        keep.swap(h->raw);
        size_t off = 0;
        for (const auto& kv : exp) {
            RawTensor t;
            t.shape = keep[kv.first].shape;
            t.data.resize(keep[kv.first].data.size());
            for (size_t i = 0; i < t.data.size(); ++i) t.data[i] = (float)(off + i + 1);
            off += t.data.size();
            h->raw[kv.first] = std::move(t);
        }
        h->h_map.clear();
        h->split_tab.clear(); h->split_pending.clear();
        if (off < (size_t(1) << 24)) {
            h->split_record = N16_SPLIT != 0;
            pack_all();
            h->split_record = false;
            h->h_map.resize(h->h_w.size());
            for (size_t i = 0; i < h->h_w.size(); ++i) h->h_map[i] = (int)h->h_w[i] - 1;
        }
        h->raw.swap(keep);
    }
    pack_all();
    if (h->d_w) { (void)hipFree(h->d_w); h->d_w = nullptr; }
// ... 1387 lines not shown
        }
    }
    {
        BwdEncodeParams p{};
        p.c = tc; p.Np = h->Np; p.Nf = h->Nf;
        p.prot_h0 = h->d_prot_h0; p.pharm_h = h->d_pharm_h; p.t = h->d_t; p.gid = h->d_gid;
        p.rec_nf = c.rec_nf; p.pharm_nf = c.pharm_nf;
        for (int nt = 0; nt < 2; ++nt) {
            const std::string pre = std::string("dynamics.") + kNtKey[nt] + "_encoder.";
            p.o_w[nt] = (int)h->flat_offset(pre + "0.weight"); p.o_b[nt] = (int)h->flat_offset(pre + "0.bias");
            p.o_lw[nt] = (int)h->flat_offset(pre + "2.weight"); p.o_lb[nt] = (int)h->flat_offset(pre + "2.bias");
        }
        p.G_h = h->t_G_h[a];
        p.B = h->B; p.onehot_flag = h->d_l0flag;
        p.Gg = (c.rec_nf <= 16 && h->Np > 0) ? h->t_Gg : nullptr;
        if (p.Gg && !enc_grouped_done) pfk_enc_group(p.G_h, h->d_prot_ptr, h->d_ptype, h->B, c.rec_nf, h->t_Gg, s);
        const int tiles = (h->Np + PFT_ROWS - 1) / PFT_ROWS + (h->Nf + PFT_ROWS - 1) / PFT_ROWS;
        rp.enc_grid = std::max(1, std::min(PFT_ENC_BLOCKS, tiles));
        pfk_bwd_encode(&p, rp.enc_grid, s);
    }
    rp.cls_mask = ~early_mask;
    pfk_train_reduce(&rp, s);
    if (early_mask) PF_HIP(h, hipStreamWaitEvent(s, h->cmp_ev[1], 0));
    hipError_t e = hipGetLastError();
    if (e != hipSuccess) PF_FAIL(h, PF_ERR_HIP, "kernel launch failed: %s", hipGetErrorString(e));
    h->tA_dirty = false;
    return PF_OK;
}

int pf_train_set_precision(pf_handle* h, int32_t precision) {
    if (!h) return PF_ERR_ARG;
    if (precision != PF_TRAIN_F32 && precision != PF_TRAIN_BF16) PF_FAIL(h, PF_ERR_ARG, "pf_train_set_precision: precision must be PF_TRAIN_F32 or PF_TRAIN_BF16");
    h->train_bf16 = precision == PF_TRAIN_BF16;
    h->t_have_fwd = false;
    h->t_have_loss = false;
    return PF_OK;
}

int pf_train_get_precision(pf_handle* h, int32_t* precision) {
    if (!h || !precision) return PF_ERR_ARG;
    *precision = h->train_bf16 ? PF_TRAIN_BF16 : PF_TRAIN_F32;
    return PF_OK;
}

int pf_debug_set_dropout_masks(pf_handle* h, const float* dev_masks) {
    if (!h) return PF_ERR_ARG;
    h->t_mask_override = dev_masks;
    return PF_OK;
}

int pf_debug_dropout_mask(pf_handle* h, int32_t layer, int32_t which, float dropout_p, uint32_t seed, float* dev_out, pf_stream stream) {
    int rc = check_ready(h, true);
    if (rc) return rc;
    if (!dev_out || layer < 0 || layer >= h->cfg.n_convs || which < 0 || which > 1) PF_FAIL(h, PF_ERR_ARG, "pf_debug_dropout_mask: bad argument");
    TrainCommon tc{};
    tc.drop_thr = dropout_p > 0.f ? (uint32_t)std::min(4294967295.0, (double)dropout_p * 4294967296.0) : 0u;
    tc.drop_scale = 1.0f / (1.0f - dropout_p);
    tc.seed = seed;
    pfk_drop_masks(&tc, (uint32_t)layer * 2u + (uint32_t)which, h->N * 144, dev_out, (hipStream_t)stream);
    return PF_OK;
}

int pf_debug_ahead(pf_handle* h, int64_t* out, pf_stream stream) {
    int rc = check_ready(h, true);
    if (rc) return rc;
    if (!out) PF_FAIL(h, PF_ERR_ARG, "pf_debug_ahead: null argument");
    out[0] = out[1] = out[2] = out[3] = 0;
    PF_HIP(h, hipStreamSynchronize((hipStream_t)stream));
    const int B = h->B;
    if (h->spec_valid && h->d_pa_same && h->d_dyn_cnt) {
        std::vector<int> cnt((size_t)5 * B), same(B);
        PF_HIP(h, hipMemcpy(cnt.data(), h->d_dyn_cnt, (size_t)5 * B * 4, hipMemcpyDeviceToHost));
        PF_HIP(h, hipMemcpy(same.data(), h->d_pa_same, (size_t)B * 4, hipMemcpyDeviceToHost));
        for (int g = 0; g < B; ++g) {
            const int64_t c = cnt[(size_t)3 * B + g];
            out[1] += c;
            out[0] += std::min<int64_t>(c, (int64_t)std::min(same[g], 1 << 26) * 16);
        }
    }
    if (h->cen_valid) { out[2] = 1; out[3] = h->Nf; }
    return PF_OK;
}

int pf_debug_pa_check(pf_handle* h, int64_t* out, pf_stream stream) {
    int rc = check_ready(h, true);
    if (rc) return rc;
    if (!out) PF_FAIL(h, PF_ERR_ARG, "pf_debug_pa_check: null argument");
    out[0] = out[1] = out[2] = 0;
    PF_HIP(h, hipStreamSynchronize((hipStream_t)stream));
    if (h->d_pa_chk) {
        unsigned long long v[3];
        PF_HIP(h, hipMemcpy(v, h->d_pa_chk, sizeof(v), hipMemcpyDeviceToHost));
        for (int k = 0; k < 3; ++k) out[k] = (int64_t)v[k];
    }
    return PF_OK;
}

int pf_debug_kernel_family(pf_handle* h, int32_t layer, int32_t* rows_per_wave) {
    if (!h || !rows_per_wave) return PF_ERR_ARG;
    if (layer == (int)h->last_family.size() + 2 && layer > 2) {
        *rows_per_wave = h->last_spec;
        return PF_OK;
    }
    if (layer == (int)h->last_family.size() + 1 && layer > 1) {
        *rows_per_wave = h->last_cen ? 1 : 0;
        return PF_OK;
    }
    if (layer == (int)h->last_family.size() && layer > 0) {
        *rows_per_wave = h->last_tail;
        return PF_OK;
    }
    if (layer < 0 || layer >= (int)h->last_family.size()) PF_FAIL(h, PF_ERR_STATE, "pf_debug_kernel_family: no dynamics call yet, or bad layer");
    *rows_per_wave = h->last_family[layer];
    return PF_OK;
}

int pf_debug_last_eps(pf_handle* h, float* dev_eps_h, float* dev_eps_x, pf_stream stream) {
    int rc = check_ready(h, true);
    if (rc) return rc;
    hipStream_t s = (hipStream_t)stream;
    if (dev_eps_h) PF_HIP(h, hipMemcpyAsync(dev_eps_h, h->d_eps_h, (size_t)h->Nf * h->cfg.pharm_nf * 4, hipMemcpyDeviceToDevice, s));
    if (dev_eps_x) PF_HIP(h, hipMemcpyAsync(dev_eps_x, h->d_eps_x, (size_t)h->Nf * 3 * 4, hipMemcpyDeviceToDevice, s));
    return PF_OK;
}

int pf_debug_xchg_timeouts(pf_handle* h, int32_t* n) {
    if (!h || !n) return PF_ERR_ARG;
    *n = 0;
    if (!h->d_xstat) return PF_OK;
    PF_HIP(h, hipDeviceSynchronize());
    PF_HIP(h, hipMemcpy(n, h->d_xstat, sizeof(int32_t), hipMemcpyDeviceToHost));
    return PF_OK;
}

int pf_debug_chain(pf_handle* h, int32_t kind, int32_t layer, int32_t sub, int32_t n_rows, const float* dev_s_in, const float* dev_v_in,
                   float* dev_s_out, float* dev_v_out, pf_stream stream) {
    if (h && !h->spec) PF_FAIL(h, PF_ERR_ARG, "%s: specialised to n_hidden_scalars 128 / vector_size 16", __func__);
    int rc = check_ready(h, false);
    if (rc) return rc;
    const pf_config& c = h->cfg;
    if (kind == 16 || kind == 17) {
        n16_refresh(h, (hipStream_t)stream);
        if (n_rows < 0 || !dev_s_in || !dev_v_in || !dev_s_out || !dev_v_out) PF_FAIL(h, PF_ERR_ARG, "pf_debug_chain: bad argument");
        if (layer < 0 || layer >= c.n_convs || sub < 0 || sub > (kind == 16 ? 3 : 1)) PF_FAIL(h, PF_ERR_ARG, "pf_debug_chain: bad layer / sub index");
        if (h->n16_msg.empty()) PF_FAIL(h, PF_ERR_STATE, "pf_debug_chain: this architecture has no n16 streams (needs n_message_gvps >= 2)");
        UnitParams p{};
        p.s_in = dev_s_in; p.v_in = dev_v_in; p.s_out = dev_s_out; p.v_out = dev_v_out;
        p.n = n_rows; p.kind = kind;
        if (kind == 16) { p.stream = h->d_w + h->n16_msg[(size_t)layer * 4 + sub]; p.n_gvps = c.n_message_gvps; p.n16_stride = (int)h->n16_msg_stride; }
        else { p.stream = h->d_w + h->n16_upd[(size_t)layer * 2 + sub]; p.n_gvps = c.n_update_gvps; p.n16_stride = (int)h->n16_upd_stride; }
        pfk_n16_unit(&p, (hipStream_t)stream);
        hipError_t e16 = hipGetLastError();
        if (e16 != hipSuccess) PF_FAIL(h, PF_ERR_HIP, "kernel launch failed: %s", hipGetErrorString(e16));
        return PF_OK;
    }
    if (kind < 0 || kind > 3 || n_rows < 0 || !dev_s_in || !dev_v_in || !dev_s_out || !dev_v_out) PF_FAIL(h, PF_ERR_ARG, "pf_debug_chain: bad argument");
    if (kind != 3 && (layer < 0 || layer >= c.n_convs)) PF_FAIL(h, PF_ERR_ARG, "pf_debug_chain: bad layer");
    if ((kind == 0 && (sub < 0 || sub > 3)) || ((kind == 1 || kind == 2) && (sub < 0 || sub > 3))) PF_FAIL(h, PF_ERR_ARG, "pf_debug_chain: bad sub index");
    if (h->rg_msg.empty()) PF_FAIL(h, PF_ERR_STATE, "pf_debug_chain: no row-group streams (weights not committed)");
    UnitParams p{};
    p.s_in = dev_s_in; p.v_in = dev_v_in; p.s_out = dev_s_out; p.v_out = dev_v_out;
    p.n = n_rows; p.kind = kind; p.pharm_nf = c.pharm_nf;
    if (kind == 0) { p.stream = h->d_w + h->rg_msg[(size_t)layer * 4 + sub]; p.n_gvps = c.n_message_gvps; }
    else if (kind == 1) {
        if (sub > 1) PF_FAIL(h, PF_ERR_ARG, "pf_debug_chain: node type 0 (prot) or 1 (pharm)");
        p.stream = h->d_w + h->rg_upd[(size_t)layer * 2 + sub]; p.n_gvps = c.n_update_gvps;
// ... 111 lines not shown
```

### pharmacophore-diffusion_amd/csrc/pf_n16.hip

```cpp
#include <hip/hip_runtime.h>
#include <type_traits>
#include <algorithm>
#include "pf_device.h"
#ifdef N16_STAMPS
#define N16_STAMP_GLOBALS 1
namespace {
__device__ unsigned long long* g_n16_stamps = nullptr;
__device__ int g_n16_stamp_off = 0;
__device__ int g_n16_stamp_kid = -1;
}
#define SB_STAMP(k)                                                                                                    \
    do {                                                                                                               \
        const int rb_ = (int)blockIdx.x - g_n16_stamp_off;                                                             \
        if ((k) < 16 && (threadIdx.x & 63) == 0 && g_n16_stamps && rb_ >= 0 && rb_ < 64 && (g_n16_stamp_kid < 0 || g_n16_stamp_kid == 3)) \
            g_n16_stamps[((size_t)rb_ * 4 + (threadIdx.x >> 6)) * 64 + 40 + (k)] = __builtin_amdgcn_s_memtime();       \
    } while (0)
#endif
#include "pf_stepbuild.h"

#include "pf_n16_core.h"

using namespace pfn16;

namespace {
// ... 287 lines not shown
    *reinterpret_cast<f32x4*>(&lds->s[((2 * wq) * 64 + lane) * 4]) = Q[0];
    *reinterpret_cast<f32x4*>(&lds->s[((2 * wq + 1) * 64 + lane) * 4]) = Q[1];
    lds_barrier();
#pragma unroll
    for (int T = 0; T < 8; ++T) {
        const f32x4 x = *reinterpret_cast<const f32x4*>(&lds->s[(T * 64 + lane) * 4]);
#pragma unroll
        for (int r = 0; r < 4; ++r) XS[4 * T + r] = x[r];
    }
}

__device__ __forceinline__ void n16_node_desc_l0(const FusedParams& f, const int node, const int nt, NodeDesc& nd) {
#pragma unroll
    for (int sl = 0; sl < 2; ++sl) {
        const int slot = sl == 0 ? 0 : (nt == 0 ? f.pp_slot : 1);
        nd.st[sl] = f.in_start[slot * f.N + node];
        nd.cn[sl] = f.in_cnt[slot * f.N + node];
        nd.gm[sl] = (sl == 0 ? f.grp : (nt == 0 ? f.grp_pa : f.grp)) - 1;
    }
}
__device__ __forceinline__ void n16_node_update_l0(const FusedParams& f, const EncodeParams& ep, N16Ring& ring, const int node, const int nt,
                                                   const NodeDesc& nd, const int pty, float (&XS)[32], float (&VB)[4], N16Lds* lds,
                                                   const int lane, const int wq, int& sk) {
    const int g = lane >> 4;
    const N16LnPre lnq = n16_ln_request(f.ln1_w[nt], f.ln1_b[nt], f.ln2_w[nt], f.ln2_b[nt], lane, wq);
    RowQ rq;
    n16_rows_load(f.msg_s, f.msg_v, f.zero_row, nd, rq, lane, wq);
    f32x4 Hq[2];
    Hq[0] = (f32x4){0.f, 0.f, 0.f, 0.f}; Hq[1] = Hq[0];
    if (nt == 0) {
        pf_gcf hp = (pf_gcf)f.htab + (f.htab_gstride ? (size_t)f.gid[node] * f.htab_gstride : 0) + (size_t)pty * PF_S + 32 * wq + 4 * g;
        Hq[0] = *reinterpret_cast<const f32x4 PF_AS1*>(hp);
        Hq[1] = *reinterpret_cast<const f32x4 PF_AS1*>(hp + 16);
    }
    float inv_norm = 1.0f;
    if (f.norm_mode == 1) inv_norm = 1.0f / f.norm_value;
    else if (f.norm_mode == 2) inv_norm = 1.0f / f.gnorm[nt * f.B + f.gid[node]];
    float H[32];
    const bool enc_here = nt != 0 && f.hcen == nullptr;
    if (nt != 0 && f.hcen != nullptr) {
        pf_gcf hp = (pf_gcf)f.hcen + (size_t)(node - ep.Np) * PF_S + 32 * wq + 4 * g;
        Hq[0] = *reinterpret_cast<const f32x4 PF_AS1*>(hp);
        Hq[1] = *reinterpret_cast<const f32x4 PF_AS1*>(hp + 16);
    }
    if (enc_here) {
        const float tt = ep.t ? ((pf_gcf)ep.t)[f.gid[node]] : ep.t_scalar;
        n16_encode_pharm(ep, (pf_gcf)ep.pharm_h + (size_t)(node - ep.Np) * ep.pharm_nf, tt, H, lds, lane, wq);
    }
    f32x4 Q[2];
    n16_rows_sum(f.msg_s, f.msg_v, f.zero_row, f.norm_mode, nd, rq, Q, VB, lds, lane, wq);
    N16_STAMP(sk, lane, wq);
    N16_CUT_AT(FUSED_CUT, 2, Q[0][0] + VB[0] + Hq[0][0], f.h_out);
#pragma unroll
    for (int r = 0; r < 4; ++r) { Q[0][r] = fmaf(Q[0][r], inv_norm, Hq[0][r]); Q[1][r] = fmaf(Q[1][r], inv_norm, Hq[1][r]); }
    n16_ln_stage(lnq, lds, lane, wq);
    n16_quarters_to_rows(Q, XS, lds, lane, wq);
    if (enc_here) {
#pragma unroll
        for (int k = 0; k < 32; ++k) XS[k] += H[k];
    }
#pragma unroll
    for (int r = 0; r < 4; ++r) VB[r] = wq < 3 ? VB[r] * inv_norm : 0.f;
    n16_layernorm<true>(nullptr, nullptr, XS, VB, lds, lane, wq, 0);
    N16_STAMP(sk, lane, wq);
    float Xr[32], Vr[4];
#pragma unroll
    for (int k = 0; k < 32; ++k) Xr[k] = XS[k];
#pragma unroll
    for (int r = 0; r < 4; ++r) Vr[r] = VB[r];
    N16In none{};
    f32x4 S[2];
    S[0] = (f32x4){0.f, 0.f, 0.f, 0.f}; S[1] = S[0];
    N16P XP;
    n16_gen_run<0>(f.n_upd, ring, XS, XP, VB, none, S, lds, lane, wq, sk);
    n16_gate_flush(VB, lds, lane, wq);
#pragma unroll
    for (int k = 0; k < 32; ++k) XS[k] += Xr[k];
#pragma unroll
    for (int r = 0; r < 4; ++r) VB[r] += Vr[r];
    n16_layernorm<true>(nullptr, nullptr, XS, VB, lds, lane, wq, 1);
}

__device__ __forceinline__ void n16_fused_store_item(const FusedParams& f, const EncodeParams& ep, N16Lds* lds, const int gq, const int part,
                                                     float (&XS)[32], float (&VB)[4], const int lane, const int wq, int& sk) {
    const int g = lane >> 4, j = lane & 15;
    const int f0 = f.pharm_ptr[gq], nf = f.pharm_ptr[gq + 1] - f0;
    const int nv = __builtin_amdgcn_readfirstlane(min(16, nf - 16 * part));
    if (nv <= 0) return;
    const int node = f.Np + f0 + 16 * part + min(j, nv - 1);
    N16Ring ring;
    ring_start(ring, f.upd_pharm + (size_t)wq * f.upd_pharm_stride, lane);
    NodeDesc nd;
    n16_node_desc_l0(f, node, 1, nd);
    n16_node_update_l0(f, ep, ring, node, 1, nd, 0, XS, VB, lds, lane, wq, sk);
    if (j < nv && wq == 0) {
        float* hp = f.h_out + (size_t)node * PF_S + 4 * g;
#pragma unroll
        for (int T = 0; T < 8; ++T) *reinterpret_cast<f32x4*>(hp + 16 * T) = (f32x4){XS[4 * T], XS[4 * T + 1], XS[4 * T + 2], XS[4 * T + 3]};
    }
    if (j < nv && wq < 3) {
        float* vp = f.v_out + (size_t)node * 48 + 12 * g + wq;
#pragma unroll
        for (int r = 0; r < 4; ++r) vp[3 * r] = VB[r];
    }
}
__device__ __forceinline__ void n16_fused_edge_item(const EdgeParams& p, const FusedParams& f, const EncodeParams& ep, N16Lds* lds, const int e,
                                                    const int src, const int dst, const int nv, const int et, float (&XS)[32],
                                                    float (&VB)[4], const int lane, const int wq, int& sk, const int4* rec = nullptr) {
    N16Ring ring;
    ring_start(ring, f.chain[et] + (size_t)wq * f.chain_stride[et], lane);
    N16Rows rw;
    rw.e = e;
    rw.dst = dst;
    const int nt = et == ET_FF ? 1 : 0;
    NodeDesc nd;
    int pty;
    if (rec) {
        rw.xs = make_float4(__builtin_bit_cast(float, rec[0].x), __builtin_bit_cast(float, rec[0].y), __builtin_bit_cast(float, rec[0].z), 0.f);
        rw.xd = make_float4(__builtin_bit_cast(float, rec[1].x), __builtin_bit_cast(float, rec[1].y), __builtin_bit_cast(float, rec[1].z), 0.f);
        nd.st[0] = rec[2].x; nd.cn[0] = rec[2].y; nd.st[1] = rec[2].z; nd.cn[1] = rec[2].w;
        nd.gm[0] = f.grp - 1; nd.gm[1] = (nt == 0 ? f.grp_pa : f.grp) - 1;
        pty = (int)((unsigned)rec[0].w >> 24);
    } else {
        rw.xs = p.xn[src]; rw.xd = p.xn[dst];
        n16_node_desc_l0(f, src, nt, nd);
        pty = nt == 0 ? f.ptype[src] : 0;
    }
    n16_node_update_l0(f, ep, ring, src, nt, nd, pty, XS, VB, lds, lane, wq, sk);
    N16_CUT_AT(FUSED_CUT, 3, XS[0] + VB[0] + rw.xs.x + rw.xd.x, f.h_out);
    f32x4 S[2];
    S[0] = (f32x4){0.f, 0.f, 0.f, 0.f}; S[1] = S[0];
    n16_edge_chain<N16_M0F>(p, ring, rw, XS, VB, S, lds, nv, lane, wq, sk);
}

__global__ __launch_bounds__(256) void k_n16_fused(const int* __restrict__ a_dyn_cnt, const int* __restrict__ a_reg, const int a_nreg,
                                                   const int a_regB, const EdgeParams p, const FusedParams f, const EncodeParams ep) {
    __shared__ N16Lds lds;
    const int lane = threadIdx.x & 63;
    const int wq = __builtin_amdgcn_readfirstlane((int)(threadIdx.x >> 6));
    const int j = lane & 15;
    int sk = 2 << 8;
    N16_STAMP(sk, lane, wq);
    float XS[32], VB[4];
    auto store_item = [&](const int gq, const int part) { n16_fused_store_item(f, ep, &lds, gq, part, XS, VB, lane, wq, sk); };
    int e0, nv, et;
    if (f.xcd_split) {
        const int b = (int)blockIdx.x, x = b & 7, kq = b >> 3;
        const int r = min(lane, a_nreg - 1);
        const int c = lane < a_nreg ? a_dyn_cnt[r] : 0;
        const int rs0 = a_reg[r];
        const int ng = (c + 15) >> 4;
        int incl = ng;
        incl += dpp_i<0x111>(incl); incl += dpp_i<0x112>(incl); incl += dpp_i<0x114>(incl); incl += dpp_i<0x118>(incl);
        incl += dpp_ir<0x142, 0xa>(incl); incl += dpp_ir<0x143, 0xc>(incl);
        const int ff_total = __builtin_amdgcn_readlane(incl, a_regB - 1), all_total = __builtin_amdgcn_readlane(incl, 63);
        int w;
        if (x < 4) {
            const int idx = 4 * kq + x;
            if (idx >= ff_total) {
                if (idx - ff_total < f.B) store_item(idx - ff_total, 0);
                return;
            }
            w = idx;
        } else {
            w = ff_total + 4 * kq + (x - 4);
            if (w >= all_total) return;
        }
        const unsigned long long m = __ballot(incl > w);
        const int l = __builtin_amdgcn_readfirstlane(__ffsll((long long)m) - 1);
        const int first = __builtin_amdgcn_readlane(incl - ng, l);
        const int cnt = __builtin_amdgcn_readlane(c, l), start = __builtin_amdgcn_readlane(rs0, l);
        et = l / a_regB;
        const int loc = (w - first) << 4;
        e0 = start + loc;
        nv = __builtin_amdgcn_readfirstlane(min(16, cnt - loc));
    } else {
    if ((int)blockIdx.x >= f.n_edge_items) {
        const int it = (int)blockIdx.x - f.n_edge_items;
        store_item(it / (PF_MAXF / 16), it % (PF_MAXF / 16));
        return;
    }
    {
        constexpr int NP = 16;
        const int w = (int)blockIdx.x;
        int first = 0, rsel = -1, cnt = 0, start = 0;
        int cs[NP], rs[NP];
#pragma unroll
        for (int k = 0; k < NP; ++k) {
            cs[k] = 0; rs[k] = 0;
            if (64 * k < a_nreg) {
                const int r = min(64 * k + lane, a_nreg - 1);
                const int c = a_dyn_cnt[r];
                rs[k] = a_reg[r];
                cs[k] = 64 * k + lane < a_nreg ? c : 0;
            }
        }
#pragma unroll
        for (int k = 0; k < NP; ++k) {
            if (64 * k < a_nreg && rsel < 0) {
                const int c = cs[k];
                const int ng = (c + 15) >> 4;
                int incl = ng;
                incl += dpp_i<0x111>(incl); incl += dpp_i<0x112>(incl); incl += dpp_i<0x114>(incl); incl += dpp_i<0x118>(incl);
                incl += dpp_ir<0x142, 0xa>(incl); incl += dpp_ir<0x143, 0xc>(incl);
                incl += first;
                const unsigned long long m = __ballot(incl > w);
                if (m) {
                    const int l = __builtin_amdgcn_readfirstlane(__ffsll((long long)m) - 1);
                    rsel = 64 * k + l;
                    first = __builtin_amdgcn_readlane(incl - ng, l);
                    cnt = __builtin_amdgcn_readlane(c, l);
                    start = __builtin_amdgcn_readlane(rs[k], l);
                } else first = __builtin_amdgcn_readlane(incl, 63);
            }
        }
        if (rsel < 0) return;
        et = rsel / a_regB;
        const int loc = (w - first) << 4;
        e0 = start + loc;
        nv = __builtin_amdgcn_readfirstlane(min(16, cnt - loc));
    }
    }
    N16_STAMP(sk, lane, wq);
    N16_CUT_AT(FUSED_CUT, 1, (float)(e0 + nv), f.h_out);
    const int e = e0 + min(j, nv - 1);
    n16_fused_edge_item(p, f, ep, &lds, e, p.esrc[e], p.edst[e], nv, et, XS, VB, lane, wq, sk);
}

__global__ __launch_bounds__(256) void k_n16_fused_u(const int* __restrict__ a_dyn_cnt, const int* __restrict__ a_esrc,
                                                     const int* __restrict__ a_edst, const int a_ff_base, const int a_pf_base,
                                                     const int a_strides, const int a_groups, const EdgeParams p,
                                                     const FusedParams f, const EncodeParams ep) {
    __shared__ N16Lds lds;
    const int lane = threadIdx.x & 63;
    const int wq = __builtin_amdgcn_readfirstlane((int)(threadIdx.x >> 6));
    const int j = lane & 15;
    int sk = 2 << 8;
    N16_STAMP(sk, lane, wq);
#ifdef N16_STAMPS
    struct WgTimes { __device__ ~WgTimes() { if (on) g_n16_stamps[(size_t)blockIdx.x * 2 + 1] = __builtin_amdgcn_s_memrealtime(); } bool on; } wgt_;
    wgt_.on = g_n16_stamp_kid == 101 && g_n16_stamps && threadIdx.x == 0 && blockIdx.x < 8192;
    if (wgt_.on) g_n16_stamps[(size_t)blockIdx.x * 2] = __builtin_amdgcn_s_memrealtime();
#endif
    float XS[32], VB[4];
    const int nffg = a_groups & 255, npfg = (a_groups >> 8) & 255, a_B = (int)((unsigned)a_groups >> 16);
    const int b = (int)blockIdx.x, x = b & 7, kq = b >> 3;
    int et, e0, cidx, k;
    if (x < 4) {
        const int idx = 4 * kq + x;
        if (idx >= a_B * nffg) {
            if (idx - a_B * nffg < a_B) n16_fused_store_item(f, ep, &lds, idx - a_B * nffg, 0, XS, VB, lane, wq, sk);
            return;
        }
        const int g = idx / nffg;
        k = idx - g * nffg;
        et = ET_FF; cidx = g; e0 = a_ff_base + g * (a_strides & 0xffff) + 16 * k;
    } else {
        const int w = 4 * kq + (x - 4);
        if (w >= a_B * npfg) return;
        const int g = w / npfg;
        k = w - g * npfg;
        et = ET_PF; cidx = a_B + g; e0 = a_pf_base + g * (int)((unsigned)a_strides >> 16) + 16 * k;
    }
    const int cnt = a_dyn_cnt[cidx];
    if (f.rec) {
        const int4* rp = f.rec + (size_t)3 * (e0 + j);
        int4 r[3] = {rp[0], rp[1], rp[2]};
        const int nv = __builtin_amdgcn_readfirstlane(min(16, cnt - 16 * k));
        if (nv <= 0) return;
        N16_STAMP(sk, lane, wq);
        const int jj = min(j, nv - 1);
        const int from = 4 * ((lane & 48) | jj);
#pragma unroll
        for (int u = 0; u < 3; ++u) {
            r[u].x = __builtin_amdgcn_ds_bpermute(from, r[u].x); r[u].y = __builtin_amdgcn_ds_bpermute(from, r[u].y);
            r[u].z = __builtin_amdgcn_ds_bpermute(from, r[u].z); r[u].w = __builtin_amdgcn_ds_bpermute(from, r[u].w);
        }
        n16_fused_edge_item(p, f, ep, &lds, e0 + jj, r[0].w & 0xffffff, r[1].w, nv, et, XS, VB, lane, wq, sk, r);
        return;
    }
    const int src_raw = a_esrc[e0 + j], dst_raw = a_edst[e0 + j];
    const int nv = __builtin_amdgcn_readfirstlane(min(16, cnt - 16 * k));
    if (nv <= 0) return;
    N16_STAMP(sk, lane, wq);
    const int jj = min(j, nv - 1);
    const int from = 4 * ((lane & 48) | jj);
    const int src = __builtin_amdgcn_ds_bpermute(from, src_raw), dst = __builtin_amdgcn_ds_bpermute(from, dst_raw);
    n16_fused_edge_item(p, f, ep, &lds, e0 + jj, src, dst, nv, et, XS, VB, lane, wq, sk);
}

struct __attribute__((aligned(16))) TailLds {
    N16Lds n;
    float ex[PF_MAXF * 4];
    float eh[PF_MAXF * 16];
    pfsb::StepBuildLds sb;
};

__device__ __forceinline__ void n16_node_desc_last(const TailParams& t, const int node, NodeDesc& nd) {
#pragma unroll
    for (int sl = 0; sl < 2; ++sl) {
        nd.st[sl] = t.in_start[sl * t.N + node];
        nd.cn[sl] = t.in_cnt[sl * t.N + node];
        nd.gm[sl] = t.grp - 1;
    }
}
template <class Hook>
__device__ __forceinline__ void n16_node_update_last(const TailParams& t, const NodeDesc& nd, N16Ring& ring, const int node, float (&XS)[32],
                                                     float (&VB)[4], N16Lds* lds, const int lane, const int wq, int& sk, Hook&& hook) {
    const int g = lane >> 4;
    const int cw = wq < 3 ? wq : 0;
    RowQ rq;
    n16_rows_load(t.msg_s, t.msg_v, t.zero_row, nd, rq, lane, wq);
    f32x4 Hq[2];
    float Vr0[4];
    {
        pf_gcf hp = (pf_gcf)t.h_in + (size_t)node * PF_S + 32 * wq + 4 * g;
        Hq[0] = *reinterpret_cast<const f32x4 PF_AS1*>(hp);
        Hq[1] = *reinterpret_cast<const f32x4 PF_AS1*>(hp + 16);
        pf_gcf vp = (pf_gcf)t.v_in + (size_t)node * 48 + 12 * g + cw;
#pragma unroll
        for (int r = 0; r < 4; ++r) Vr0[r] = vp[3 * r];
    }
    float inv_norm = 1.0f;
    if (t.norm_mode == 1) inv_norm = 1.0f / t.norm_value;
    else if (t.norm_mode == 2) inv_norm = 1.0f / t.gnorm[1 * t.B + t.gid[node]];
    hook(0);
    f32x4 Q[2];
    n16_rows_sum(t.msg_s, t.msg_v, t.zero_row, t.norm_mode, nd, rq, Q, VB, lds, lane, wq);
    N16_STAMP(sk, lane, wq);
    N16_CUT_AT(TAIL_CUT, 1, Q[0][0] + VB[0] + Hq[0][0] + Vr0[0], t.eps_h);
#pragma unroll
    for (int r = 0; r < 4; ++r) { Q[0][r] = fmaf(Q[0][r], inv_norm, Hq[0][r]); Q[1][r] = fmaf(Q[1][r], inv_norm, Hq[1][r]); }
    n16_quarters_to_rows(Q, XS, lds, lane, wq);
#pragma unroll
    for (int r = 0; r < 4; ++r) VB[r] = wq < 3 ? fmaf(VB[r], inv_norm, Vr0[r]) : 0.f;
    n16_layernorm(t.ln1_w, t.ln1_b, XS, VB, lds, lane, wq);
    hook(1);
    float Xr[32], Vr[4];
#pragma unroll
    for (int k = 0; k < 32; ++k) Xr[k] = XS[k];
#pragma unroll
    for (int r = 0; r < 4; ++r) Vr[r] = VB[r];
    N16In none{};
    f32x4 S[2];
    S[0] = (f32x4){0.f, 0.f, 0.f, 0.f}; S[1] = S[0];
    N16P XP;
    n16_gen_run<0>(t.n_upd, ring, XS, XP, VB, none, S, lds, lane, wq, sk);
    n16_gate_flush(VB, lds, lane, wq);
#pragma unroll
    for (int k = 0; k < 32; ++k) XS[k] += Xr[k];
#pragma unroll
    for (int r = 0; r < 4; ++r) VB[r] += Vr[r];
    n16_layernorm(t.ln2_w, t.ln2_b, XS, VB, lds, lane, wq);
}

__global__ __launch_bounds__(256) void k_n16_tail(const int* __restrict__ a_prot_ptr, const int* __restrict__ a_pharm_ptr,
                                                  const int* __restrict__ a_reg, const int a_B, const int a_Np_tot,
                                                  const TailParams t, const StepParams sp, const BuildParams bp) {
    __shared__ TailLds L;
    const int lane = threadIdx.x & 63;
// ... 66 lines not shown
    __shared__ N16Lds lds;
    const int lane = threadIdx.x & 63;
    const int wq = __builtin_amdgcn_readfirstlane((int)(threadIdx.x >> 6));
    const int e0 = 16 * (int)blockIdx.x;
    const int nv = __builtin_amdgcn_readfirstlane(min(16, p.n - e0));
    if (nv <= 0) return;
    const int g = lane >> 4, j = lane & 15;
    const int row = e0 + min(j, nv - 1);
    const bool msg = p.kind == 16;
    int sk = 4 << 8;
    N16_STAMP(sk, lane, wq);
    const int sw = msg ? 144 : 128, vw = msg ? 51 : 48, v0 = msg ? 3 : 0;
    N16Ring ring;
    ring_start(ring, (pf_gcf)p.stream + (size_t)wq * p.n16_stride, lane);
    float XS[32], VB[4];
    f32x4 S[2];
    S[0] = (f32x4){0.f, 0.f, 0.f, 0.f}; S[1] = S[0];
#pragma unroll
    for (int T = 0; T < 8; ++T)
#pragma unroll
        for (int r = 0; r < 4; ++r) XS[4 * T + r] = p.s_in[(size_t)row * sw + 16 * T + 4 * g + r];
#pragma unroll
    for (int r = 0; r < 4; ++r) VB[r] = wq < 3 ? p.v_in[(size_t)row * vw + v0 + (4 * g + r) * 3 + wq] : 0.f;
    N16In in;
#pragma unroll
    for (int r = 0; r < 4; ++r) in.rb[r] = msg ? p.s_in[(size_t)row * sw + 128 + 4 * g + r] : 0.f;
#pragma unroll
    for (int c = 0; c < 3; ++c) in.xh[c] = msg ? p.v_in[(size_t)row * vw + c] : 0.f;
    N16P XP;
    if (msg) {
        constexpr int OFF1 = n16_sched(N16_M0F).nq % N16_D;
        n16_split_rows(XS, XP);
        n16_block<N16_M0F, 0, false, true, false, false>(ring, XS, XP, VB, in, S, &lds, lane, wq, sk);
        for (int gi = 1; gi + 1 < p.n_gvps; ++gi) n16_block<N16_GEN, OFF1, false, true, true, false>(ring, XS, XP, VB, in, S, &lds, lane, wq, sk);
        n16_block<N16_GEN, OFF1, true, true, true>(ring, XS, XP, VB, in, S, &lds, lane, wq, sk);
    } else {
        n16_gen_run<0, false>(p.n_gvps - 1, ring, XS, XP, VB, in, S, &lds, lane, wq, sk);
        if (p.n_gvps > 1) n16_block<N16_GEN, 0, true, true, true>(ring, XS, XP, VB, in, S, &lds, lane, wq, sk);
        else { n16_split_rows(XS, XP); n16_block<N16_GEN, 0, true, true, false>(ring, XS, XP, VB, in, S, &lds, lane, wq, sk); }
    }
    N16_STAMP(sk, lane, wq);
    if (j < nv) {
        float* so = p.s_out + (size_t)row * 128 + 32 * wq + 4 * g;
        *reinterpret_cast<f32x4*>(so) = S[0];
        *reinterpret_cast<f32x4*>(so + 16) = S[1];
        if (wq < 3) {
#pragma unroll
            for (int r = 0; r < 4; ++r) p.v_out[(size_t)row * 48 + (4 * g + r) * 3 + wq] = VB[r];
        }
    }
}

}

extern "C" {
void pfk_n16_edge(const EdgeParams* p, const EncodeParams* enc, int layer0, hipStream_t s) {
    if (p->ntiles == 0) return;
    const int grid = p->nreg > 0 ? p->ngroups_sel : p->ntiles * 2;
    if (grid <= 0) return;
    const EncodeParams noenc{};
    if (layer0 && p->uni_s2g != 0) {
        const int B = p->regB;
        const int nstat = B * (((p->uni_s2g >> 16) & 7) + ((p->uni_s2g >> 19) & 7) + ((p->uni_s2g >> 22) & 7));
        hipLaunchKernelGGL(k_n16_edge_u, dim3(nstat + p->uni_pa_groups), dim3(256), 0, s, p->dyn_cnt, p->esrc, p->edst, p->uni_base[0],
                           p->uni_base[1], p->uni_base[2], p->uni_s01, p->uni_s2g, p->reg, *p, *enc);
        return;
    }
    if (layer0) hipLaunchKernelGGL((k_n16_edge<true>), dim3(grid), dim3(256), 0, s, p->dyn_cnt, p->reg, p->nreg, p->regB, p->pa_abs, *p, *enc);
    else hipLaunchKernelGGL((k_n16_edge<false>), dim3(grid), dim3(256), 0, s, p->dyn_cnt, p->reg, p->nreg, p->regB, p->pa_abs, *p, noenc);
}
#ifdef N16_STAMPS
int pfk_n16_set_stamp_buffer(unsigned long long* dev, int off) {
    (void)hipMemcpyToSymbol(HIP_SYMBOL(g_n16_stamp_off), &off, sizeof(off));
    return (int)hipMemcpyToSymbol(HIP_SYMBOL(g_n16_stamps), &dev, sizeof(dev));
}
int pfk_n16_set_stamp_kernel(int kid) { return (int)hipMemcpyToSymbol(HIP_SYMBOL(g_n16_stamp_kid), &kid, sizeof(kid)); }
#endif
#ifdef N16_TRACE
int pfk_n16_set_trace_buffer(unsigned long long* dev) { return (int)hipMemcpyToSymbol(HIP_SYMBOL(g_n16_trace), &dev, sizeof(dev)); }
#endif
void pfk_n16_fused(const EdgeParams* p, const FusedParams* f, const EncodeParams* enc, hipStream_t s) {
    if (f->uni_groups != 0) {
        const int nffg = f->uni_groups & 255, npfg = (f->uni_groups >> 8) & 255;
        const int grid_u = 8 * std::max((f->B * nffg + f->B + 3) / 4, (f->B * npfg + 3) / 4);
        if (grid_u > 0)
            hipLaunchKernelGGL(k_n16_fused_u, dim3(grid_u), dim3(256), 0, s, p->dyn_cnt, p->esrc, p->edst, f->uni_ff_base, f->uni_pf_base,
                               f->uni_strides, f->uni_groups | (f->B << 16), *p, *f, *enc);
        return;
    }
    int grid = f->n_edge_items + f->B * (PF_MAXF / 16);
    if (f->xcd_split) grid = 8 * std::max((f->nff_cap + f->B + 3) / 4, (f->npf_cap + 3) / 4);
    if (grid <= 0) return;
    hipLaunchKernelGGL(k_n16_fused, dim3(grid), dim3(256), 0, s, p->dyn_cnt, p->reg, p->nreg, p->regB, *p, *f, *enc);
}
void pfk_n16_tail(const TailParams* t, const StepParams* sp, const BuildParams* bp, hipStream_t s) {
    if (sp->B <= 0) return;
    hipLaunchKernelGGL(k_n16_tail, dim3(sp->B), dim3(256), 0, s, bp->prot_ptr, bp->pharm_ptr, bp->reg, bp->B, bp->Np_tot, *t, *sp, *bp);
}
void pfk_n16_unit(const UnitParams* p, hipStream_t s) {
    if (p->n <= 0) return;
    hipLaunchKernelGGL(k_n16_unit, dim3((p->n + 15) / 16), dim3(256), 0, s, *p);
}
}
```

### pharmacophore-diffusion_amd/csrc/pf_rg.hip

```cpp
#include <hip/hip_runtime.h>
#include <type_traits>
#include <algorithm>
#include "pf_device.h"
#ifdef PF_HSB_STAMPS
__device__ unsigned long long* g_hsb_stamps = nullptr;
#define PF_HSB_SLOTS 24
#define SB_STAMP(k) do { const int kk_ = (k) == 100 ? 2 : (k) == 101 ? 3 : (k) == 8 ? 4 : (k) == 10 ? 5 : (k) == 14 ? 6 : (k) == 11 ? 7 : (k) == 9 ? 8 : (k) == 20 ? 9 : (k) == 21 ? 10 : (k) == 12 ? 11 : (k) == 13 ? 12 : (k) == 15 ? 13 : (k) >= 30 && (k) < 40 ? (k) - 16 : -1; \
        const bool who_ = (k) == 21 ? (int)threadIdx.x == (int)blockDim.x - 64 : threadIdx.x == 0; \
        if (kk_ >= 0 && who_ && g_hsb_stamps) g_hsb_stamps[blockIdx.x * PF_HSB_SLOTS + kk_] = __builtin_amdgcn_s_memrealtime(); } while (0)
#endif
#include "pf_stepbuild.h"
#include "pf_cenhoist.h"
#include "pf_n16_core.h"
#include "pf_train.h"

typedef float f32x4 __attribute__((ext_vector_type(4)));

namespace {

template <int I, int N, class F>
__device__ __forceinline__ void static_for(F&& f) {
    if constexpr (I < N) {
        f(std::integral_constant<int, I>{});
        static_for<I + 1, N>(f);
// ... 1019 lines not shown
    const int nv = __builtin_amdgcn_readfirstlane(min(4, a_n - base));
    if (nv <= 0) return;
    NodeTile t{};
    t.n0 = a_n0 + (base & ~31); t.n = 32; t.ntype = 1; t.cnt_idx = -1; t.rel = 0; t.ids = 0;
    NodeParams q = p;
    q.in_start = a_in_start; q.in_cnt = a_in_cnt;
    const EncodeParams noenc{};
    rg_node_item<false, 1, true, 2, false>(t, base & 31, nv, nv, 1, item, wq, lds_all[0], q, hp, noenc, lane, nullptr, nullptr, 0, [](const int) {});
}

#ifdef PF_HSB_STAMPS
#define HSB_STAMP(k) do { if (threadIdx.x == 0 && g_hsb_stamps) g_hsb_stamps[blockIdx.x * PF_HSB_SLOTS + (k)] = __builtin_amdgcn_s_memrealtime(); } while (0)
#else
#define HSB_STAMP(k)
#endif
__device__ __forceinline__ bool pa_spec_item(const int w, const EdgeParams& es, const EncodeParams& ees, pfn16::N16Lds* lds, const int lane,
                                             const int wq) {
    const int a_B = es.regB;
    if (a_B <= 0) return false;
    const int r = 3 * a_B + min(lane, a_B - 1);
    const int c = lane < a_B ? es.cnt_snap[lane] : 0;
    const int rs = es.reg[r];
    const int ng = (c + 15) >> 4;
    int incl = ng;
    incl += pfn16::dpp_i<0x111>(incl); incl += pfn16::dpp_i<0x112>(incl); incl += pfn16::dpp_i<0x114>(incl); incl += pfn16::dpp_i<0x118>(incl);
    incl += pfn16::dpp_ir<0x142, 0xa>(incl); incl += pfn16::dpp_ir<0x143, 0xc>(incl);
    const unsigned long long m = __ballot(incl > w);
    if (!m) return false;
    const int l = __builtin_amdgcn_readfirstlane(__ffsll((long long)m) - 1);
    const int first = __builtin_amdgcn_readlane(incl - ng, l);
    const int cnt = __builtin_amdgcn_readlane(c, l), start = __builtin_amdgcn_readlane(rs, l);
    const int loc = (w - first) << 4;
    const int nv = __builtin_amdgcn_readfirstlane(min(16, cnt - loc));
    if (nv <= 0) return false;
    if (es.pa_gstamp && threadIdx.x == 0) es.pa_gstamp[(start + loc) >> 4] = es.pa_serial;
    const int e = start + loc + min(lane & 15, nv - 1);
    int sk = 0;
    pfn16::n16_edge_item<N16_M0H>(es, ees, lds, e, es.esrc[e], es.edst[e], nv, (int)ET_PP, lane, wq, sk);
    return true;
}

__global__ __launch_bounds__(256) void k_pa_spec(const int a_after, const int a_k, const int a_frac, int* a_word, const EdgeParams es,
                                                 const EncodeParams ees) {
    __shared__ pfn16::N16Lds lds;
    const int lane = threadIdx.x & 63;
    const int wq = __builtin_amdgcn_readfirstlane((int)(threadIdx.x >> 6));
    const int w = (int)blockIdx.x;
    int k;
    if (a_after) k = __builtin_amdgcn_readfirstlane(*a_word);
    else {
        k = a_k;
        if (a_frac > 0) {
            const int a_B = es.regB;
            int ng = lane < a_B ? (es.cnt_snap[lane] + 15) >> 4 : 0;
            for (int o = 32; o > 0; o >>= 1) ng += __shfl_xor(ng, o);
            k = __builtin_amdgcn_readfirstlane((int)(((long long)ng * a_frac) >> 8));
        }
        if (w == 0 && threadIdx.x == 0) *a_word = k;
    }
    if (a_after ? w < k : w >= k) return;
    pa_spec_item(w, es, ees, &lds, lane, wq);
}

__global__ __launch_bounds__(64) void k_pa_check(const int* __restrict__ dyn_cnt, const int* __restrict__ cnt_snap, const int* __restrict__ reg,
                                                 const int* __restrict__ pa_same, const int* __restrict__ gstamp, const int serial, const int B,
                                                 unsigned long long* out) {
    const int g = (int)threadIdx.x;
    if (g >= B) return;
    const int ng = (dyn_cnt[3 * B + g] + 15) >> 4;
    const int keep = max(min(pa_same[g], ng), 0);
    const int s0 = reg[3 * B + g] >> 4;
    int bad = 0, po = 0, pn = 0;
    for (int j = 0; j < keep; ++j) bad += gstamp[s0 + j] != serial;
    for (int k = 0; k < g; ++k) { po += (cnt_snap[k] + 15) >> 4; pn += (dyn_cnt[3 * B + k] + 15) >> 4; }
    if (bad) atomicAdd(&out[0], (unsigned long long)bad);
    if (keep) atomicAdd(&out[1], (unsigned long long)keep);
    if (keep && po != pn) atomicAdd(&out[2], (unsigned long long)keep);
}

struct __attribute__((aligned(16))) RgHsbLds {
    union { RgLds item[2][1]; pfsb::StepBuildLds sb; pfch::CenHoistLds ch; pfn16::N16Lds n16; };
};
struct HsbPlain {};
struct HsbExtra { CenHoistParams cp; int gs; EdgeParams es; EncodeParams ees; };
template <class Extra>
__global__ __launch_bounds__(256) void k_rg_node_hs_build(const int* __restrict__ a_in_start, const int* __restrict__ a_in_cnt, const int a_n0,
                                                          const int a_n, const int a_xcd_n, const int a_gh, const NodeParams p,
                                                          const HeadParams hp, const StepParams sp, const BuildParams bp, int* xstat,
                                                          const int poll_sleep, const int avoid, const int poll_max, const int a_gb,
                                                          const Extra ex) {
    constexpr bool EXTRA = std::is_same<Extra, HsbExtra>::value;
    __shared__ RgHsbLds L;
    const int lane = threadIdx.x & 63;
    const int wq = __builtin_amdgcn_readfirstlane((int)(threadIdx.x >> 6));
    const int b = (int)blockIdx.x;
    HSB_STAMP(0);
    if (b < a_gh) {
        int wgi = b;
        if (a_xcd_n > 0) {
            const int x = b & 7;
            if (x >= a_xcd_n) return;
            wgi = (b >> 3) * a_xcd_n + x;
        }
        if (wq >= 2) return;
        const int item = wgi, half = wq;
        const int base = 4 * item;
        const int nv = __builtin_amdgcn_readfirstlane(min(4, a_n - base));
        if (nv <= 0) return;
        NodeTile t{};
        t.n0 = a_n0 + (base & ~31); t.n = 32; t.ntype = 1; t.cnt_idx = -1; t.rel = 0; t.ids = 0;
        NodeParams q = p;
        q.in_start = a_in_start; q.in_cnt = a_in_cnt;
        const EncodeParams noenc{};
        rg_node_item<false, 1, true, 2, false>(t, base & 31, nv, nv, 1, item, half, L.item[0], q, hp, noenc, lane, nullptr, nullptr, 0,
                                               [](const int) {});
        HSB_STAMP(1);
        return;
    }
    if constexpr (EXTRA) {
    const int a_gs = ex.gs;
    const EdgeParams& es = ex.es;
    const EncodeParams& ees = ex.ees;
    const CenHoistParams& cp = ex.cp;
    if (b >= a_gh + a_gb && b < a_gh + a_gb + a_gs) {
        int w = b - a_gh - a_gb;
        if (a_xcd_n > 0) {
            const int x = b & 7;
            if (x < a_xcd_n) return;
            w = (w >> 3) * (8 - a_xcd_n) + (x - a_xcd_n);
        }
        if (pa_spec_item(w, es, ees, &L.n16, lane, wq)) { HSB_STAMP(1); }
        return;
    }
    if (b >= a_gh + a_gb + a_gs) {
        int it = b - a_gh - a_gb - a_gs;
        if (a_xcd_n > 0) {
            const int x = b & 7;
            if (x < a_xcd_n) return;
            it = (it >> 3) * (8 - a_xcd_n) + (x - a_xcd_n);
        }
        pfch::cen_hoist_item(it, cp, xstat, poll_sleep, poll_max, L.ch);
        HSB_STAMP(1);
        return;
    }
    }
    int g = b - a_gh;
    if (avoid > 0) {
        const int x = (b - a_gh) & 7;
        if (x < avoid) return;
        g = ((b - a_gh) >> 3) * (8 - avoid) + (x - avoid);
    }
    if (g >= bp.B) return;
    pfsb::step_build_wait_body<256>(g, bp.prot_ptr, bp.pharm_ptr, bp.reg, bp.B, bp.Np_tot, sp, bp, hp.xchg, xstat, L.sb, poll_sleep, poll_max);
    HSB_STAMP(1);
}

struct __attribute__((aligned(16))) RgTailLds {
    RgLds item[2][1];
    float ex[PF_MAXF * 4];
    float eh[PF_MAXF * 16];
    pfsb::StepBuildLds sb;
};
__global__ __launch_bounds__(256) void k_rg_tail(const int* __restrict__ a_prot_ptr, const int* __restrict__ a_pharm_ptr,
                                                 const int* __restrict__ a_reg, const int a_B, const int a_Np_tot,
                                                 const NodeParams p, const HeadParams hp, const StepParams sp, const BuildParams bp) {
    __shared__ RgTailLds L;
    const int lane = threadIdx.x & 63;
    const int wq = __builtin_amdgcn_readfirstlane((int)(threadIdx.x >> 6));
    const int pair = wq >> 1, half = wq & 1;
    const int gq = (int)blockIdx.x;
    pfsb::SbPre<256> pre;
    pfsb::sb_load_a<256>(pre, gq, a_prot_ptr, a_pharm_ptr, a_reg, a_B, a_Np_tot, bp);
    const int f0 = pre.f0, Nf = pre.Nf;
    bool c_loaded = false;
    if (Nf == 0) pfsb::sb_load_b<256>(pre, a_Np_tot, sp, bp);
    const EncodeParams noenc{};
    for (int base8 = 0; base8 < Nf; base8 += 8) {
        const int here = min(8, Nf - base8);
        const int mine = here - 4 * pair;
        NodeTile t{};
        t.n0 = a_Np_tot + f0 + base8 + (mine > 0 ? 4 * pair : 0);
        t.n = 4; t.ntype = 1; t.cnt_idx = -1; t.rel = 0; t.ids = 0;
        const int nv = __builtin_amdgcn_readfirstlane(mine > 0 ? min(4, mine) : min(4, here));
        const int nv_store = __builtin_amdgcn_readfirstlane(max(min(4, mine), 0));
        rg_node_item<false, 1, true, 2, false>(t, 0, nv, nv_store, 1, 2 * gq + pair, half, L.item[pair], p, hp, noenc, lane, L.ex, L.eh,
                                               f0, [&](const int phase) {
            if (c_loaded) return;
            if (phase == 0) pfsb::sb_load_b<256>(pre, a_Np_tot, sp, bp);
            else { pfsb::sb_load_c<256>(pre, bp); c_loaded = true; }
        });
        pfsb::sb_lds_barrier();
    }
    if (!c_loaded) pfsb::sb_load_c<256>(pre, bp);
    float ex[3], eh[pfsb::SB_MAXNF];
    const int fme = min((int)threadIdx.x, PF_MAXF - 1);
#pragma unroll
    for (int c = 0; c < 3; ++c) ex[c] = L.ex[fme * 4 + c];
#pragma unroll
    for (int k = 0; k < pfsb::SB_MAXNF; ++k) eh[k] = L.eh[fme * 16 + k];
    pfsb::sb_finish<256>(pre, ex, eh, gq, sp, bp, L.sb);
}

template <bool SAVE>
__global__ __launch_bounds__(64) void k_rg_unit(const UnitParams p) {
    constexpr int RG = 1, D = RgDepth<1>::D;
    __shared__ RgLds lds[1];
    const int lane = threadIdx.x & 63;
    const int e0 = 4 * (int)blockIdx.x;
    const int nv = __builtin_amdgcn_readfirstlane(min(4, p.n - e0));
    if (nv <= 0) return;
    const int a = lane >> 2, i = lane & 3, g = lane >> 4, q = a & 3, u = lane & 15;
    const int row = e0 + min(i, nv - 1);
    const bool msg = p.kind == 0;
    const int sw = msg ? 144 : 128, vw = msg ? 51 : 48, v0 = msg ? 3 : 0;
    float X[RG][8], Va[RG][4], R[RG], XH[RG];
#pragma unroll
    for (int m = 0; m < 8; ++m) X[0][m] = p.s_in[(size_t)row * sw + 8 * a + m];
#pragma unroll
    for (int tt = 0; tt < 4; ++tt) Va[0][tt] = g < 3 ? p.v_in[(size_t)row * vw + v0 + (q + 4 * tt) * 3 + g] : 0.f;
    R[0] = msg ? p.s_in[(size_t)row * sw + 128 + a] : 0.f;
    XH[0] = (msg && g < 3) ? p.v_in[(size_t)row * vw + g] : 0.f;
    if (p.kind == 2) {
        rg_layernorm<RG>((pf_gcf)p.ln_w, (pf_gcf)p.ln_b, X, Va, lane);
        if (i < nv) {
#pragma unroll
            for (int m = 0; m < 8; ++m) p.s_out[(size_t)row * 128 + 8 * a + m] = X[0][m];
            if (g < 3) {
#pragma unroll
                for (int tt = 0; tt < 4; ++tt) p.v_out[(size_t)row * 48 + (q + 4 * tt) * 3 + g] = Va[0][tt];
            }
        }
        return;
    }
// ... 119 lines not shown
    for (int k = 0; k < PF_S; ++k) {
        a0 = fmaf(p.src[L0H_WHT + k * PF_S + f], hs[k], a0);
        a2 = fmaf(p.src[L0H_WHT_PF + k * PF_S + f], hs[k], a2);
    }
    float* out = p.ptab + ((size_t)it * L0_NTAB * p.rec_nf + ty) * PF_S + f;
    out[0] = a0;
    out[(size_t)p.rec_nf * PF_S] = a0 + p.src[L0H_B + f];
    out[(size_t)2 * p.rec_nf * PF_S] = a2 + p.src[L0H_B_PF + f];
    out[(size_t)3 * p.rec_nf * PF_S] = hs[f];
}
__global__ __launch_bounds__(256) void k_l0_types(const L0HoistParams p) {
    const int n = blockIdx.x * 256 + threadIdx.x;
    int* eorig = reinterpret_cast<int*>(p.zs);
    for (int e = n; e < p.Epp; e += gridDim.x * 256) eorig[e] = e;
    if (n >= p.Np) return;
    int ty = -1, bad = 0;
    for (int k = 0; k < p.rec_nf; ++k) {
        const float x = p.prot_h0[(size_t)n * p.rec_nf + k];
        if (x == 1.0f) { if (ty >= 0) bad = 1; ty = k; }
        else if (x != 0.0f) bad = 1;
    }
    if (ty < 0) { bad = 1; ty = 0; }
    p.ptype[n] = ty;
    if (bad) atomicOr(p.flag, 1);
}

}

extern "C" {
#ifdef PF_HSB_STAMPS
int pfk_hsb_set_stamp_buffer(unsigned long long* dev) { return (int)hipMemcpyToSymbol(HIP_SYMBOL(g_hsb_stamps), &dev, sizeof(dev)); }
#endif
#ifdef PF_STAMPS
int pfk_rg_set_stamp_buffer(unsigned long long* dev) { g_rg_stamp_host_buf = dev; unsigned long long* z = nullptr; return (int)hipMemcpyToSymbol(HIP_SYMBOL(g_rg_stamps), &z, sizeof(z)); }
int pfk_rg_set_stamp_offset(int off) { return (int)hipMemcpyToSymbol(HIP_SYMBOL(g_rg_stamp_off), &off, sizeof(off)); }
void pfk_rg_set_stamp_which(int which) { g_rg_stamp_which = which; g_rg_stamp_seen = 0; }
#endif
void pfk_l0_hoist(const L0HoistParams* p, int what, hipStream_t s) {
    if (what == 0) {
        hipLaunchKernelGGL(k_l0_consts, dim3(1), dim3(64), 0, s, *p);
        if (p->Epp > 0) hipLaunchKernelGGL(k_l0_zs, dim3(std::min(p->Epp, 8192)), dim3(128), 0, s, *p);
    } else if (what == 1) {
        if (p->nt > 0) hipLaunchKernelGGL(k_l0_ptab, dim3(p->nt * p->rec_nf), dim3(128), 0, s, *p);
    } else hipLaunchKernelGGL(k_l0_types, dim3(std::max(1, (p->Np + 255) / 256)), dim3(256), 0, s, *p);
}
void pfk_rg_edge(const EdgeParams* p, const EncodeParams* enc, int layer0, int rg, int split, int rgp, hipStream_t s) {
    if (p->ntiles == 0) return;
#ifdef PF_STAMPS
    rg_stamp_arm(s);
#endif
    const int per = 32 / (4 * rg);
    const int grid = p->nreg > 0 ? (p->ngroups_sel > 0 ? p->ngroups_sel : (rg == 1 ? p->ngroups4 : p->ngroups8)) : p->ntiles * per;
    if (grid == 0) return;
    const EncodeParams noenc{};
    const EncodeParams& ep = (layer0 && enc) ? *enc : noenc;
    const int grid4 = grid <= 256 ? grid : (grid + 1023) / 1024 * 256;
    const bool quad = grid <= RG_QUAD_MAX;
    if (!layer0 || split || !p->zs) rgp = 0;
#define PF_RG_EDGE(L0_, RG_, W_, P_, GRID_) hipLaunchKernelGGL((k_rg_edge<L0_, RG_, W_, P_>), dim3(GRID_), dim3(64 * W_), 0, s, *p, ep)
    if (p->sv_z != nullptr) {
#define PF_RG_EDGE_SV(L0_, RG_) hipLaunchKernelGGL((k_rg_edge<L0_, RG_, 1, 0, true>), dim3(grid), dim3(64), 0, s, *p, ep)
        if (layer0) { if (rg == 1) PF_RG_EDGE_SV(true, 1); else PF_RG_EDGE_SV(true, 2); }
        else { if (rg == 1) PF_RG_EDGE_SV(false, 1); else PF_RG_EDGE_SV(false, 2); }
#undef PF_RG_EDGE_SV
        return;
    }
    if (rg == 1 && split) { if (layer0) PF_RG_EDGE(true, 1, 2, 0, grid); else PF_RG_EDGE(false, 1, 2, 0, grid); }
    else if (!layer0) {
        if (rg == 1 && quad) PF_RG_EDGE(false, 1, 4, 0, grid4);
        else if (rg == 1) PF_RG_EDGE(false, 1, 1, 0, grid);
        else if (quad) PF_RG_EDGE(false, 2, 4, 0, grid4);
        else PF_RG_EDGE(false, 2, 1, 0, grid);
    } else if (rg == 1 && rgp == 2) { if (quad) PF_RG_EDGE(true, 1, 4, 2, grid4); else PF_RG_EDGE(true, 1, 1, 2, grid); }
    else if (rg == 1) { if (quad) PF_RG_EDGE(true, 1, 4, 1, grid4); else PF_RG_EDGE(true, 1, 1, 1, grid); }
    else { if (quad) PF_RG_EDGE(true, 2, 4, 2, grid4); else PF_RG_EDGE(true, 2, 1, 2, grid); }
#undef PF_RG_EDGE
}
void pfk_rg_tail(const NodeParams* p, const HeadParams* hp, const StepParams* sp, const BuildParams* bp, hipStream_t s) {
    if (sp->B <= 0) return;
    hipLaunchKernelGGL(k_rg_tail, dim3(sp->B), dim3(256), 0, s, bp->prot_ptr, bp->pharm_ptr, bp->reg, bp->B, bp->Np_tot, *p, *hp, *sp, *bp);
}
void pfk_rg_node_hs_build(const NodeParams* p, const HeadParams* hp, const StepParams* sp, const BuildParams* bp, int* xstat, int poll_sleep,
                          int avoid, int poll_max, const CenHoistParams* cp, const EdgeParams* es, const EncodeParams* ees, int spec_groups,
                          hipStream_t s) {
    if (sp->B <= 0 || p->st_n <= 0) return;
    const int items = (p->st_n + 3) / 4, wgs = items;
    const int gh = p->xcd_n > 0 ? (wgs + p->xcd_n - 1) / p->xcd_n * 8 : wgs;
    if (p->xcd_n <= 0 || avoid < 0 || avoid > 7) avoid = 0;
    const int gb = avoid > 0 ? (sp->B + (8 - avoid) - 1) / (8 - avoid) * 8 : sp->B;
    int gs = (es && ees && spec_groups > 0 && es->regB <= 64) ? spec_groups : 0;
    int pad = 0;
    if (gs && p->xcd_n > 0 && p->xcd_n < 8) {
        pad = (8 - ((gh + gb) & 7)) & 7;
        gs = (gs + (8 - p->xcd_n) - 1) / (8 - p->xcd_n) * 8;
    }
    int gc = (cp && cp->on) ? (cp->Nf + pfch::CH_ROWS - 1) / pfch::CH_ROWS : 0;
    int pad2 = 0;
    if (gc && p->xcd_n > 0 && p->xcd_n < 8) {
        pad2 = (8 - ((gh + gb + pad + gs) & 7)) & 7;
        gc = (gc + (8 - p->xcd_n) - 1) / (8 - p->xcd_n) * 8;
    }
    const int pm = poll_max > 0 ? poll_max : pfsb::SB_XCHG_POLLS;
    if (gc == 0 && gs == 0) {
        hipLaunchKernelGGL(k_rg_node_hs_build<HsbPlain>, dim3(gh + gb), dim3(256), 0, s, p->in_start, p->in_cnt, p->st_n0, p->st_n, p->xcd_n, gh,
                           *p, *hp, *sp, *bp, xstat, poll_sleep, avoid, pm, gb, HsbPlain{});
        return;
    }
    HsbExtra ex{};
    if (gc) ex.cp = *cp;
    ex.gs = gs + pad2;
    if (gs) { ex.es = *es; ex.ees = *ees; }
    hipLaunchKernelGGL(k_rg_node_hs_build<HsbExtra>, dim3(gh + gb + pad + gs + pad2 + gc), dim3(256), 0, s, p->in_start, p->in_cnt, p->st_n0, p->st_n,
                       p->xcd_n, gh, *p, *hp, *sp, *bp, xstat, poll_sleep, avoid, pm, gb + pad, ex);
}
void pfk_pa_spec(const EdgeParams* es, const EncodeParams* ees, int groups, int after, int k, int frac, int* word, hipStream_t s) {
    if (groups <= 0 || es->regB <= 0 || es->regB > 64) return;
    hipLaunchKernelGGL(k_pa_spec, dim3(groups), dim3(256), 0, s, after, k, frac, word, *es, *ees);
}
void pfk_pa_check(const int* dyn_cnt, const int* cnt_snap, const int* reg, const int* pa_same, const int* gstamp, int serial, int B,
                  unsigned long long* out, hipStream_t s) {
    if (B <= 0 || B > 64) return;
    hipLaunchKernelGGL(k_pa_check, dim3(1), dim3(64), 0, s, dyn_cnt, cnt_snap, reg, pa_same, gstamp, serial, B, out);
}
void pfk_rg_unit(const UnitParams* p, hipStream_t s) {
    if (p->n <= 0) return;
    if (p->sv_z != nullptr && p->kind == 3) hipLaunchKernelGGL(k_rg_unit<true>, dim3((p->n + 3) / 4), dim3(64), 0, s, *p);
    else hipLaunchKernelGGL(k_rg_unit<false>, dim3((p->n + 3) / 4), dim3(64), 0, s, *p);
}
void pfk_rg_node(const NodeParams* p, const HeadParams* hp, const EncodeParams* enc, int layer0, int rg, int split, hipStream_t s) {
    if (p->ntiles == 0) return;
#ifdef PF_STAMPS
    rg_stamp_arm(s);
#endif
    const int per = 32 / (4 * rg);
    const HeadParams none{};
    const bool head = hp != nullptr;
    const HeadParams& h = head ? *hp : none;
    const int grid = p->ntiles * per;
    const EncodeParams noenc{};
    const EncodeParams& ep = (layer0 && enc) ? *enc : noenc;
    if (head && !layer0 && rg == 1 && split && p->st_n > 0 && p->sv_z == nullptr) {
        const int items = (p->st_n + 3) / 4;
        const int g2 = p->xcd_n > 0 ? (items + p->xcd_n - 1) / p->xcd_n * 8 : items;
        hipLaunchKernelGGL(k_rg_node_hs, dim3(g2), dim3(128), 0, s, p->in_start, p->in_cnt, p->st_n0, p->st_n, p->xcd_n, *p, h);
        return;
    }
    const int grid4 = grid <= 256 ? grid : (grid + 1023) / 1024 * 256;
    const bool quad = grid <= RG_QUAD_MAX;
    if (p->sv_z != nullptr && !head) {
#define PF_RG_NODE_SV(L0_, RG_) hipLaunchKernelGGL((k_rg_node<L0_, RG_, false, 1, true>), dim3(grid), dim3(64), 0, s, p->tiles, p->ntiles, p->dyn_cnt, *p, h, ep)
        if (layer0) { if (rg == 1) PF_RG_NODE_SV(true, 1); else PF_RG_NODE_SV(true, 2); }
        else { if (rg == 1) PF_RG_NODE_SV(false, 1); else PF_RG_NODE_SV(false, 2); }
#undef PF_RG_NODE_SV
        return;
    }
#define PF_RG_NODE(L0_, RG_, HEAD_, W_, GRID_) hipLaunchKernelGGL((k_rg_node<L0_, RG_, HEAD_, W_>), dim3(GRID_), dim3(64 * W_), 0, s, p->tiles, p->ntiles, p->dyn_cnt, *p, h, ep)
#define PF_RG_NODE2(RG_, W_, GRID_)                                                                      \
    do {                                                                                                 \
        if (head) { if (layer0) PF_RG_NODE(true, RG_, true, W_, GRID_); else PF_RG_NODE(false, RG_, true, W_, GRID_); }   \
        else { if (layer0) PF_RG_NODE(true, RG_, false, W_, GRID_); else PF_RG_NODE(false, RG_, false, W_, GRID_); }      \
    } while (0)
    if (rg == 1 && split) PF_RG_NODE2(1, 2, p->xcd_n > 0 ? (grid + p->xcd_n - 1) / p->xcd_n * 8 : grid);
    else if (rg == 1 && quad) PF_RG_NODE2(1, 4, grid4);
    else if (rg == 1) PF_RG_NODE2(1, 1, grid);
    else if (quad) PF_RG_NODE2(2, 4, grid4);
    else PF_RG_NODE2(2, 1, grid);
#undef PF_RG_NODE2
#undef PF_RG_NODE
}
}
```

### pharmacophore-diffusion_amd/engine.py

```python
import ctypes
from typing import Dict, Optional

import torch

from . import _lib as L


def _stream_ptr():
    return ctypes.c_void_p(torch.cuda.current_stream().cuda_stream)


def _dptr(t: Optional[torch.Tensor]):
    if t is None:
        return None
    assert t.is_cuda and t.is_contiguous(), "device tensors must be contiguous CUDA/HIP tensors"
    return ctypes.c_void_p(t.data_ptr())


def _i32_host(t: torch.Tensor):
    import numpy as np
    a = t.detach().cpu().numpy() if isinstance(t, torch.Tensor) else np.asarray(t)
    return np.ascontiguousarray(a, dtype=np.int32)


# ... 286 lines not shown
            tx = torch.empty(n_steps + 1, self.Nf, 3, device=self.device)
            th = torch.empty(n_steps + 1, self.Nf, self.pharm_nf, device=self.device)
        with torch.cuda.device(self.device):
            self._ck(self.lib.pf_sample(self._h, n_steps, coef_arr, _dptr(nz), _dptr(com), int(ep_coord), int(ep_feat),
                                        float(feat_norm_constant), _dptr(x0), _dptr(h0), _dptr(tx), _dptr(th),
                                        _stream_ptr()), "pf_sample")
        return (x0, h0, tx, th) if trajectory else (x0, h0)

    def sample_status(self):
        n = ctypes.c_int32()
        self._ck(self.lib.pf_sample_status(self._h, ctypes.byref(n)), "pf_sample_status")

    def get_edges(self, etype: int):
        with torch.cuda.device(self.device):
            n = self._ck(self.lib.pf_debug_get_edges(self._h, etype, None, None, 0, _stream_ptr()), "pf_debug_get_edges")
            src = torch.zeros(max(n, 1), dtype=torch.int32)
            dst = torch.zeros(max(n, 1), dtype=torch.int32)
            self._ck(self.lib.pf_debug_get_edges(self._h, etype, src.data_ptr(), dst.data_ptr(), n, _stream_ptr()),
                     "pf_debug_get_edges")
        return src[:n].long(), dst[:n].long()

    def conv_layer(self, layer, prot_x, pharm_x, h_prot, v_prot, h_pharm, v_pharm):
        a = [_f32(t, self.device) for t in (prot_x, pharm_x, h_prot, v_prot, h_pharm, v_pharm)]
        outs = [torch.empty_like(a[2]), torch.empty_like(a[3]), torch.empty_like(a[4]), torch.empty_like(a[5])]
        with torch.cuda.device(self.device):
            self._ck(self.lib.pf_debug_conv_layer(self._h, layer, *[_dptr(t) for t in a], *[_dptr(t) for t in outs],
                                                  _stream_ptr()), "pf_debug_conv_layer")
        return outs

    def work(self):
        w = self.work_detail()
        return w["flops"], w["bytes"], w["edges"]

    def work_detail(self):
        fl, by, ex = ctypes.c_double(), ctypes.c_double(), ctypes.c_double()
        ne = (ctypes.c_int64 * 4)()
        el = (ctypes.c_int64 * max(int(self.cfg.n_convs), 1))()
        with torch.cuda.device(self.device):
            self._ck(self.lib.pf_debug_work(self._h, ctypes.byref(fl), ctypes.byref(by), ne, ctypes.byref(ex), el,
                                            _stream_ptr()), "pf_debug_work")
        return {"flops": fl.value, "bytes": by.value, "edges": list(ne), "executed_flops": ex.value,
                "executed_edges_per_layer": list(el)}

    def counts(self):
        out = (ctypes.c_int64 * 8)()
        with torch.cuda.device(self.device):
            self._ck(self.lib.pf_debug_counts(self._h, out, _stream_ptr()), "pf_debug_counts")
        return dict(zip(("ff", "pf", "fp", "pp", "pa", "active_atoms", "centers", "atoms"), list(out)))

    def kernel_family(self, layer: int = 0) -> int:
        r = ctypes.c_int32()
        self._ck(self.lib.pf_debug_kernel_family(self._h, int(layer), ctypes.byref(r)), "pf_debug_kernel_family")
        return int(r.value)

    def last_eps(self):
        eh = torch.empty(self.Nf, self.pharm_nf, device=self.device); ex = torch.empty(self.Nf, 3, device=self.device)
        with torch.cuda.device(self.device):
            self._ck(self.lib.pf_debug_last_eps(self._h, _dptr(eh), _dptr(ex), _stream_ptr()), "pf_debug_last_eps")
        return eh, ex

    def xchg_timeouts(self) -> int:
        r = ctypes.c_int32()
        self._ck(self.lib.pf_debug_xchg_timeouts(self._h, ctypes.byref(r)), "pf_debug_xchg_timeouts")
        return int(r.value)

    def xchg_fault(self, drop_word: bool, poll_max: int = 0):
        self._ck(self.lib.pf_debug_xchg_fault(self._h, int(bool(drop_word)), int(poll_max)), "pf_debug_xchg_fault")

    def ahead(self):
        out = (ctypes.c_int64 * 4)()
        with torch.cuda.device(self.device):
            self._ck(self.lib.pf_debug_ahead(self._h, out, _stream_ptr()), "pf_debug_ahead")
        return dict(zip(("pa_skipped", "pa_ahead", "center_hoist", "centers"), list(out)))

    def pa_check_counts(self):
        out = (ctypes.c_int64 * 3)()
        with torch.cuda.device(self.device):
            self._ck(self.lib.pf_debug_pa_check(self._h, out, _stream_ptr()), "pf_debug_pa_check")
        return dict(zip(("violations", "checked", "exposed"), list(out)))

    def pa_check(self) -> int:
        return self.pa_check_counts()["violations"]

    def l0_hoist(self) -> int:
        r = ctypes.c_int32()
        self._ck(self.lib.pf_debug_l0_hoist(self._h, ctypes.byref(r)), "pf_debug_l0_hoist")
        return int(r.value)

    def debug_chain(self, kind: int, layer: int, sub: int, s_in: torch.Tensor, v_in: torch.Tensor):
        s_in = s_in.to(self.device, torch.float32).contiguous()
        v_in = v_in.to(self.device, torch.float32).contiguous()
        n = s_in.shape[0]
        if kind == 3:
            s_out = torch.empty(n, self.cfg.pharm_nf, device=self.device)
            v_out = torch.empty(n, 3, device=self.device)
        else:
            s_out = torch.empty(n, 128, device=self.device)
            v_out = torch.empty(n, 16, 3, device=self.device)
        with torch.cuda.device(self.device):
            self._ck(self.lib.pf_debug_chain(self._h, int(kind), int(layer), int(sub), int(n), _dptr(s_in), _dptr(v_in),
                                             _dptr(s_out), _dptr(v_out), _stream_ptr()), "pf_debug_chain")
        return s_out, v_out

    KERNEL_CLASSES = ("encode", "build_edges", "edge_msg", "node_update", "noise_head", "step_update", "edge_msg_coop",
                      "node_update_coop", "edge_msg_last")

    def profile_enable(self, mask: int):
        self._ck(self.lib.pf_profile_enable(self._h, mask), "pf_profile_enable")

    TRAIN_KERNEL_CLASSES = ("bwd_head", "bwd_node", "bwd_edge_level", "bwd_rest")

    def profile_read_train(self):
        ms = (ctypes.c_double * 4)()
        n = (ctypes.c_int64 * 4)()
        with torch.cuda.device(self.device):
            self._ck(self.lib.pf_profile_read_train(self._h, ms, n, _stream_ptr()), "pf_profile_read_train")
        return {k: (ms[i], n[i]) for i, k in enumerate(self.TRAIN_KERNEL_CLASSES)}

    def profile_read(self):
        ms = (ctypes.c_double * 9)()
        n = (ctypes.c_int64 * 9)()
        with torch.cuda.device(self.device):
            self._ck(self.lib.pf_profile_read(self._h, ms, n, _stream_ptr()), "pf_profile_read")
        return {k: (ms[i], n[i]) for i, k in enumerate(self.KERNEL_CLASSES)}
```

Baseline: 686,300 sample-steps/s.

## Prefetch next-stage weight images into L2 using idle workgroups on free XCD slots

Adds extra workgroups to the fused n16 edge kernel and the merged head/step-build kernel. Their only job is to stream the weight images the following kernels will need (edge chains, pharm update, head update) through L2, so those kernels start with warm caches. The number of warm rows is capped by how many CUs per XCD appear free. The change also passes uniform pharm counts and the rec pointer as kernel arguments, and moves the early return after the bpermute in the uniform kernel. The cost is extra memory traffic and workgroups that may compete with real work or evict useful cache lines.

```diff
diff --git a/include/pfdyn.h b/include/pfdyn.h
--- a/include/pfdyn.h
+++ b/include/pfdyn.h
@@ -146,6 +146,7 @@
 int pf_debug_kernel_family(pf_handle* h, int32_t layer, int32_t* rows_per_wave);
 int pf_debug_ahead(pf_handle* h, int64_t* out , pf_stream stream);
 int pf_debug_pa_check(pf_handle* h, int64_t* violations , pf_stream stream);
+int pf_debug_l2_warm(pf_handle* h, int32_t out[4]);
 int pf_debug_xchg_timeouts(pf_handle* h, int32_t* n);
 int pf_debug_xchg_fault(pf_handle* h, int32_t drop_word, int32_t poll_max);
 int pf_debug_last_eps(pf_handle* h, float* dev_eps_h , float* dev_eps_x , pf_stream stream);
diff --git a/pharmacophore-diffusion_amd/_lib.py b/pharmacophore-diffusion_amd/_lib.py
--- a/pharmacophore-diffusion_amd/_lib.py
+++ b/pharmacophore-diffusion_amd/_lib.py
@@ -77,6 +77,7 @@
     "pf_debug_xchg_fault": (ctypes.c_int, [_P, _I32, _I32]),
     "pf_debug_ahead": (ctypes.c_int, [_P, ctypes.POINTER(_I64), _P]),
     "pf_debug_pa_check": (ctypes.c_int, [_P, ctypes.POINTER(_I64), _P]),
+    "pf_debug_l2_warm": (ctypes.c_int, [_P, ctypes.POINTER(_I32)]),
     "pf_debug_l0_hoist": (ctypes.c_int, [_P, ctypes.POINTER(ctypes.c_int32)]),
     "pf_debug_chain": (ctypes.c_int, [_P, _I32, _I32, _I32, _I32, _P, _P, _P, _P, _P]),
 }
diff --git a/pharmacophore-diffusion_amd/csrc/pf_device.h b/pharmacophore-diffusion_amd/csrc/pf_device.h
--- a/pharmacophore-diffusion_amd/csrc/pf_device.h
+++ b/pharmacophore-diffusion_amd/csrc/pf_device.h
@@ -209,6 +209,34 @@
     int n16_stride;
 };
 
+#define PF_WARM_MAX 4
+#define PF_XCD_CUS 32
+struct WarmImage { const float* base; unsigned bytes; };
+static inline int pf_warm_rows(const int busy) {
+    const int free_cus = PF_XCD_CUS - busy;
+    return free_cus < 0 ? 0 : (free_cus < PF_WARM_MAX ? free_cus : PF_WARM_MAX);
+}
+#ifdef __HIPCC__
+__device__ __forceinline__ void pf_l2_warm(const WarmImage im, const int i, const int n) {
+    typedef float warm_f4 __attribute__((ext_vector_type(4)));
+    const unsigned nu = im.bytes >> 4;
+    const unsigned step = 256u * (unsigned)n;
+    const warm_f4 PF_AS1* src = reinterpret_cast<const warm_f4 PF_AS1*>((pf_gcf)im.base);
+    unsigned u = 256u * (unsigned)i + threadIdx.x;
+    for (; u + 15u * step < nu; u += 16u * step) {
+        warm_f4 v[16];
+#pragma unroll
+        for (int k = 0; k < 16; ++k) v[k] = src[u + (unsigned)k * step];
+#pragma unroll
+        for (int k = 0; k < 16; ++k) asm volatile("" ::"v"(v[k]));
+    }
+    for (; u < nu; u += step) {
+        const warm_f4 v = src[u];
+        asm volatile("" ::"v"(v));
+    }
+}
+#endif
+
 struct NodeParams {
     const NodeTile* tiles;
     int ntiles;
@@ -261,6 +289,8 @@
     int uni_ff_base, uni_pf_base, uni_strides, uni_groups;
     const int4* rec;
     const float* hcen;
+    int uni_nf;
+    int warm_n; WarmImage warm[3];
 };
 
 struct TailParams {
diff --git a/pharmacophore-diffusion_amd/csrc/pf_host.cpp b/pharmacophore-diffusion_amd/csrc/pf_host.cpp
--- a/pharmacophore-diffusion_amd/csrc/pf_host.cpp
+++ b/pharmacophore-diffusion_amd/csrc/pf_host.cpp
@@ -33,7 +33,7 @@
 void pfk_rg_unit(const UnitParams* p, hipStream_t s);
 void pfk_rg_node_hs_build(const NodeParams* p, const HeadParams* hp, const StepParams* sp, const BuildParams* bp, int* xstat, int poll_sleep,
                           int avoid, int poll_max, const CenHoistParams* cp, const EdgeParams* es, const EncodeParams* ees, int spec_groups,
-                          hipStream_t s);
+                          const WarmImage* warm, int* warm_wgs, hipStream_t s);
 void pfk_n16_edge(const EdgeParams* p, const EncodeParams* enc, int layer0, hipStream_t s);
 void pfk_pa_spec(const EdgeParams* es, const EncodeParams* ees, int groups, int after, int k, int frac, int* word, hipStream_t s);
 void pfk_pa_check(const int* dyn_cnt, const int* cnt_snap, const int* reg, const int* pa_same, const int* gstamp, int serial, int B,
@@ -263,6 +263,9 @@
     bool cen_valid = false; float cen_t = 0.f; uint64_t cen_wver = 0;
     bool last_cen = false;
     bool pa_spec = true;
+    bool l2_warm = true;
+    int last_warm[4] = {0, 0, 0, 0};
+    size_t rgs_head_size = 0;
     bool spec_valid = false; float spec_t = 0.f; uint64_t spec_wver = 0;
     int step_id = 2;
     int *d_pa_stamp = nullptr, *d_pa_same = nullptr;
@@ -330,6 +333,7 @@
         if (const char* e = getenv("PFDYN_NO_L0_HOIST")) l0_hoist = atoi(e) == 0;
         if (const char* e = getenv("PFDYN_NO_CENTER_HOIST")) cen_hoist = atoi(e) == 0;
         if (const char* e = getenv("PFDYN_NO_PA_SPEC")) pa_spec = atoi(e) == 0;
+        if (const char* e = getenv("PFDYN_NO_L2_WARM")) l2_warm = atoi(e) == 0;
         if (const char* e = getenv("PFDYN_PA_SPEC_SPLIT")) pa_spec_split = !strcmp(e, "mid") ? -1 : (!strcmp(e, "step") ? -2 : std::max(atoi(e), 0));
         if (const char* e = getenv("PFDYN_PA_CHECK")) pa_check = atoi(e) != 0;
         if (const char* e = getenv("PFDYN_NO_POCKET_SHARE")) share_disable = atoi(e) != 0;
@@ -1262,6 +1266,20 @@
             fz.uni_ff_base = h->h_reg[0]; fz.uni_pf_base = h->h_reg[(size_t)h->B];
             fz.uni_strides = stride[0] | (stride[1] << 16); fz.uni_groups = ((cap[0] + 15) / 16) | (((cap[1] + 15) / 16) << 8);
         }
+        if (uni) {
+            fz.uni_nf = h->max_nf;
+            for (int g = 0; g < h->B; ++g) if (h->h_pharm_ptr[(size_t)g + 1] - h->h_pharm_ptr[(size_t)g] != h->max_nf) fz.uni_nf = 0;
+        }
+        h->last_warm[2] = h->last_warm[3] = 0;
+        if (fz.xcd_split && h->l2_warm) {
+            const int rows = uni ? std::max((h->B * (fz.uni_groups & 255) + h->B + 3) / 4, (h->B * ((fz.uni_groups >> 8) & 255) + 3) / 4)
+                                 : std::max((fz.nff_cap + h->B + 3) / 4, (fz.npf_cap + 3) / 4);
+            fz.warm_n = pf_warm_rows(rows);
+            const size_t fl[3] = {4 * h->n16_fused_stride[0], 4 * h->n16_fused_stride[1], 4 * h->n16_upd_stride};
+            const float* base[3] = {fz.chain[ET_FF], fz.chain[ET_PF], fz.upd_pharm};
+            for (int k = 0; k < 3; ++k) { fz.warm[k].base = base[k]; fz.warm[k].bytes = (unsigned)(fl[k] * sizeof(float)); }
+            if (fz.warm_n > 0) { h->last_warm[2] = 8 * fz.warm_n; h->last_warm[3] = (int)((fl[0] + fl[1] + fl[2]) * sizeof(float)); }
+        }
         h->last_family[l] = 17;
         { ProfScope ps(h, pf_handle::K_EDGE_LAST, s); pfk_n16_fused(&e, &fz, &dc.ep, s); }
     }
@@ -1349,7 +1367,10 @@
         const int frac = h->pa_spec_split == -1 ? 128 : (h->pa_spec_split == -2 ? (int)((((uint32_t)h->pa_serial * 2654435761u) >> 16) & 255) + 1 : 0);
         pfk_pa_spec(&es, &ees, spec_groups, 0, std::max(h->pa_spec_split, 0), frac, h->d_pa_cnt + h->B, s);
     }
-    { ProfScope ps(h, pf_handle::K_HEAD, s); pfk_rg_node_hs_build(&n, &hp, dc.step, &bpn, h->d_xstat, h->pol.xchg_sleep, h->pol.hsb_avoid, h->xchg_poll_max, &cp, &es, &ees, split ? 0 : spec_groups, s); }
+    WarmImage warm{n.rgs_upd[1], (unsigned)(h->rgs_head_size * sizeof(float))};
+    int warm_wgs = 0;
+    { ProfScope ps(h, pf_handle::K_HEAD, s); pfk_rg_node_hs_build(&n, &hp, dc.step, &bpn, h->d_xstat, h->pol.xchg_sleep, h->pol.hsb_avoid, h->xchg_poll_max, &cp, &es, &ees, split ? 0 : spec_groups, h->l2_warm ? &warm : nullptr, &warm_wgs, s); }
+    h->last_warm[0] = warm_wgs; h->last_warm[1] = warm_wgs ? (int)warm.bytes : 0;
     if (split) pfk_pa_spec(&es, &ees, spec_groups, 1, 0, 0, h->d_pa_cnt + h->B, s);
     build_done(h, sn, with_rec);
     h->tail_done = true; h->last_tail = 2;
@@ -1420,6 +1441,7 @@
     const pf_config& c = h->cfg;
     h->tail_done = false; h->last_tail = 0;
     DynCall dc{};
+    for (int k = 0; k < 4; ++k) h->last_warm[k] = 0;
     dc.h = h; dc.s = s; dc.eps_h = eps_h; dc.eps_x = eps_x; dc.t_scalar = t_scalar; dc.train = train; dc.step = step;
     dc.cen_have = !train && h->cen_valid && h->edges_built && t_scalar != nullptr && *t_scalar == h->cen_t && h->cen_wver == h->w_version;
     h->cen_valid = false; h->last_cen = false;
@@ -1738,6 +1760,7 @@
                     if (!tail) h->rgs_upd[(size_t)l * 2 + nt] = flush();
                 }
             st.resize(st.size() + (size_t)RG_TAIL_PAD * 256, 0.f);
+            h->rgs_head_size = st.size();
             h->rgs_upd[(size_t)(c.n_convs - 1) * 2 + 1] = flush();
         }
         h->n16_begin = h->spec ? h->h_w.size() : 0;
@@ -3291,6 +3314,12 @@
     return PF_OK;
 }
 
+int pf_debug_l2_warm(pf_handle* h, int32_t out[4]) {
+    if (!h) return PF_ERR_ARG;
+    if (!out) PF_FAIL(h, PF_ERR_ARG, "pf_debug_l2_warm: null argument");
+    for (int k = 0; k < 4; ++k) out[k] = h->last_warm[k];
+    return PF_OK;
+}
 int pf_debug_pa_check(pf_handle* h, int64_t* out, pf_stream stream) {
     int rc = check_ready(h, true);
     if (rc) return rc;
diff --git a/pharmacophore-diffusion_amd/csrc/pf_n16.hip b/pharmacophore-diffusion_amd/csrc/pf_n16.hip
--- a/pharmacophore-diffusion_amd/csrc/pf_n16.hip
+++ b/pharmacophore-diffusion_amd/csrc/pf_n16.hip
@@ -393,9 +393,10 @@
 }
 
 __device__ __forceinline__ void n16_fused_store_item(const FusedParams& f, const EncodeParams& ep, N16Lds* lds, const int gq, const int part,
-                                                     float (&XS)[32], float (&VB)[4], const int lane, const int wq, int& sk) {
+                                                     float (&XS)[32], float (&VB)[4], const int lane, const int wq, int& sk,
+                                                     const int uni_nf = 0) {
     const int g = lane >> 4, j = lane & 15;
-    const int f0 = f.pharm_ptr[gq], nf = f.pharm_ptr[gq + 1] - f0;
+    const int f0 = uni_nf > 0 ? gq * uni_nf : f.pharm_ptr[gq], nf = uni_nf > 0 ? uni_nf : f.pharm_ptr[gq + 1] - f0;
     const int nv = __builtin_amdgcn_readfirstlane(min(16, nf - 16 * part));
     if (nv <= 0) return;
     const int node = f.Np + f0 + 16 * part + min(j, nv - 1);
@@ -444,6 +445,10 @@
     n16_edge_chain<N16_M0F>(p, ring, rw, XS, VB, S, lds, nv, lane, wq, sk);
 }
 
+__device__ __forceinline__ void n16_fused_warm(const FusedParams& f, const int x, const int wi) {
+#pragma unroll 1
+    for (int k = x < 4 ? 0 : 1; k < 3; k += 2) pf_l2_warm(f.warm[k], wi, f.warm_n);
+}
 __global__ __launch_bounds__(256) void k_n16_fused(const int* __restrict__ a_dyn_cnt, const int* __restrict__ a_reg, const int a_nreg,
                                                    const int a_regB, const EdgeParams p, const FusedParams f, const EncodeParams ep) {
     __shared__ N16Lds lds;
@@ -457,6 +462,13 @@
     int e0, nv, et;
     if (f.xcd_split) {
         const int b = (int)blockIdx.x, x = b & 7, kq = b >> 3;
+        if (f.warm_n > 0) {
+            const int wi = kq - (x < 4 ? (f.nff_cap + f.B + 3) / 4 : (f.npf_cap + 3) / 4);
+            if (wi >= 0) {
+                if (wi < f.warm_n) n16_fused_warm(f, x, wi);
+                return;
+            }
+        }
         const int r = min(lane, a_nreg - 1);
         const int c = lane < a_nreg ? a_dyn_cnt[r] : 0;
         const int rs0 = a_reg[r];
@@ -538,9 +550,9 @@
     n16_fused_edge_item(p, f, ep, &lds, e, p.esrc[e], p.edst[e], nv, et, XS, VB, lane, wq, sk);
 }
 
-__global__ __launch_bounds__(256) void k_n16_fused_u(const int* __restrict__ a_dyn_cnt, const int* __restrict__ a_esrc,
-                                                     const int* __restrict__ a_edst, const int a_ff_base, const int a_pf_base,
-                                                     const int a_strides, const int a_groups, const EdgeParams p,
+__global__ __launch_bounds__(256) void k_n16_fused_u(const int* __restrict__ a_dyn_cnt, const int4* __restrict__ a_rec, const int a_ff_base,
+                                                     const int a_pf_base, const int a_strides, const int a_groups,
+                                                     const int* __restrict__ a_esrc, const int* __restrict__ a_edst, const EdgeParams p,
                                                      const FusedParams f, const EncodeParams ep) {
     __shared__ N16Lds lds;
     const int lane = threadIdx.x & 63;
@@ -554,13 +566,15 @@
     if (wgt_.on) g_n16_stamps[(size_t)blockIdx.x * 2] = __builtin_amdgcn_s_memrealtime();
 #endif
     float XS[32], VB[4];
-    const int nffg = a_groups & 255, npfg = (a_groups >> 8) & 255, a_B = (int)((unsigned)a_groups >> 16);
+    const int nffg = a_groups & 255, npfg = (a_groups >> 8) & 255, a_B = (a_groups >> 16) & 255, a_nf = (int)((unsigned)a_groups >> 24);
     const int b = (int)blockIdx.x, x = b & 7, kq = b >> 3;
     int et, e0, cidx, k;
     if (x < 4) {
         const int idx = 4 * kq + x;
         if (idx >= a_B * nffg) {
-            if (idx - a_B * nffg < a_B) n16_fused_store_item(f, ep, &lds, idx - a_B * nffg, 0, XS, VB, lane, wq, sk);
+            const int wi = kq - (a_B * nffg + a_B + 3) / 4;
+            if (idx - a_B * nffg < a_B) n16_fused_store_item(f, ep, &lds, idx - a_B * nffg, 0, XS, VB, lane, wq, sk, a_nf);
+            else if (wi >= 0 && wi < f.warm_n) n16_fused_warm(f, x, wi);
             return;
         }
         const int g = idx / nffg;
@@ -568,25 +582,37 @@
         et = ET_FF; cidx = g; e0 = a_ff_base + g * (a_strides & 0xffff) + 16 * k;
     } else {
         const int w = 4 * kq + (x - 4);
-        if (w >= a_B * npfg) return;
+        if (w >= a_B * npfg) {
+            const int wi = kq - (a_B * npfg + 3) / 4;
+            if (wi >= 0 && wi < f.warm_n) n16_fused_warm(f, x, wi);
+            return;
+        }
         const int g = w / npfg;
         k = w - g * npfg;
         et = ET_PF; cidx = a_B + g; e0 = a_pf_base + g * (int)((unsigned)a_strides >> 16) + 16 * k;
     }
     const int cnt = a_dyn_cnt[cidx];
-    if (f.rec) {
-        const int4* rp = f.rec + (size_t)3 * (e0 + j);
+#ifdef N16_REC_KERNARG
+    const int4* const rec = f.rec;
+#else
+    const int4* const rec = a_rec;
+#endif
+    if (rec) {
+        const int4* rp = rec + (size_t)3 * (e0 + j);
         int4 r[3] = {rp[0], rp[1], rp[2]};
         const int nv = __builtin_amdgcn_readfirstlane(min(16, cnt - 16 * k));
+#ifdef N16_REC_KERNARG
         if (nv <= 0) return;
-        N16_STAMP(sk, lane, wq);
-        const int jj = min(j, nv - 1);
+#endif
+        const int jj = min(j, max(nv, 1) - 1);
         const int from = 4 * ((lane & 48) | jj);
 #pragma unroll
         for (int u = 0; u < 3; ++u) {
             r[u].x = __builtin_amdgcn_ds_bpermute(from, r[u].x); r[u].y = __builtin_amdgcn_ds_bpermute(from, r[u].y);
             r[u].z = __builtin_amdgcn_ds_bpermute(from, r[u].z); r[u].w = __builtin_amdgcn_ds_bpermute(from, r[u].w);
         }
+        if (nv <= 0) return;
+        N16_STAMP(sk, lane, wq);
         n16_fused_edge_item(p, f, ep, &lds, e0 + jj, r[0].w & 0xffffff, r[1].w, nv, et, XS, VB, lane, wq, sk, r);
         return;
     }
@@ -819,14 +845,14 @@
 void pfk_n16_fused(const EdgeParams* p, const FusedParams* f, const EncodeParams* enc, hipStream_t s) {
     if (f->uni_groups != 0) {
         const int nffg = f->uni_groups & 255, npfg = (f->uni_groups >> 8) & 255;
-        const int grid_u = 8 * std::max((f->B * nffg + f->B + 3) / 4, (f->B * npfg + 3) / 4);
+        const int grid_u = 8 * (std::max((f->B * nffg + f->B + 3) / 4, (f->B * npfg + 3) / 4) + f->warm_n);
         if (grid_u > 0)
-            hipLaunchKernelGGL(k_n16_fused_u, dim3(grid_u), dim3(256), 0, s, p->dyn_cnt, p->esrc, p->edst, f->uni_ff_base, f->uni_pf_base,
-                               f->uni_strides, f->uni_groups | (f->B << 16), *p, *f, *enc);
+            hipLaunchKernelGGL(k_n16_fused_u, dim3(grid_u), dim3(256), 0, s, p->dyn_cnt, f->rec, f->uni_ff_base, f->uni_pf_base, f->uni_strides,
+                               f->uni_groups | (f->B << 16) | (f->uni_nf << 24), p->esrc, p->edst, *p, *f, *enc);
         return;
     }
     int grid = f->n_edge_items + f->B * (PF_MAXF / 16);
-    if (f->xcd_split) grid = 8 * std::max((f->nff_cap + f->B + 3) / 4, (f->npf_cap + 3) / 4);
+    if (f->xcd_split) grid = 8 * (std::max((f->nff_cap + f->B + 3) / 4, (f->npf_cap + 3) / 4) + f->warm_n);
     if (grid <= 0) return;
     hipLaunchKernelGGL(k_n16_fused, dim3(grid), dim3(256), 0, s, p->dyn_cnt, p->reg, p->nreg, p->regB, *p, *f, *enc);
 }
diff --git a/pharmacophore-diffusion_amd/csrc/pf_rg.hip b/pharmacophore-diffusion_amd/csrc/pf_rg.hip
--- a/pharmacophore-diffusion_amd/csrc/pf_rg.hip
+++ b/pharmacophore-diffusion_amd/csrc/pf_rg.hip
@@ -1125,7 +1125,10 @@
     union { RgLds item[2][1]; pfsb::StepBuildLds sb; pfch::CenHoistLds ch; pfn16::N16Lds n16; };
 };
 struct HsbPlain {};
-struct HsbExtra { CenHoistParams cp; int gs; EdgeParams es; EncodeParams ees; };
+struct HsbExtra {
+    CenHoistParams cp; int gs; EdgeParams es; EncodeParams ees;
+    int gw; WarmImage warm;
+};
 template <class Extra>
 __global__ __launch_bounds__(256) void k_rg_node_hs_build(const int* __restrict__ a_in_start, const int* __restrict__ a_in_cnt, const int a_n0,
                                                           const int a_n, const int a_xcd_n, const int a_gh, const NodeParams p,
@@ -1160,13 +1163,19 @@
         HSB_STAMP(1);
         return;
     }
+    int gh2 = a_gh;
     if constexpr (EXTRA) {
+    gh2 += ex.gw;
+    if (b < gh2) {
+        if ((b & 7) < a_xcd_n) pf_l2_warm(ex.warm, (b - a_gh) >> 3, ex.gw >> 3);
+        return;
+    }
     const int a_gs = ex.gs;
     const EdgeParams& es = ex.es;
     const EncodeParams& ees = ex.ees;
     const CenHoistParams& cp = ex.cp;
-    if (b >= a_gh + a_gb && b < a_gh + a_gb + a_gs) {
-        int w = b - a_gh - a_gb;
+    if (b >= gh2 + a_gb && b < gh2 + a_gb + a_gs) {
+        int w = b - gh2 - a_gb;
         if (a_xcd_n > 0) {
             const int x = b & 7;
             if (x < a_xcd_n) return;
@@ -1175,8 +1184,8 @@
         if (pa_spec_item(w, es, ees, &L.n16, lane, wq)) { HSB_STAMP(1); }
         return;
     }
-    if (b >= a_gh + a_gb + a_gs) {
-        int it = b - a_gh - a_gb - a_gs;
+    if (b >= gh2 + a_gb + a_gs) {
+        int it = b - gh2 - a_gb - a_gs;
         if (a_xcd_n > 0) {
             const int x = b & 7;
             if (x < a_xcd_n) return;
@@ -1187,11 +1196,11 @@
         return;
     }
     }
-    int g = b - a_gh;
+    int g = b - gh2;
     if (avoid > 0) {
-        const int x = (b - a_gh) & 7;
+        const int x = (b - gh2) & 7;
         if (x < avoid) return;
-        g = ((b - a_gh) >> 3) * (8 - avoid) + (x - avoid);
+        g = ((b - gh2) >> 3) * (8 - avoid) + (x - avoid);
     }
     if (g >= bp.B) return;
     pfsb::step_build_wait_body<256>(g, bp.prot_ptr, bp.pharm_ptr, bp.reg, bp.B, bp.Np_tot, sp, bp, hp.xchg, xstat, L.sb, poll_sleep, poll_max);
@@ -1477,7 +1486,8 @@
 }
 void pfk_rg_node_hs_build(const NodeParams* p, const HeadParams* hp, const StepParams* sp, const BuildParams* bp, int* xstat, int poll_sleep,
                           int avoid, int poll_max, const CenHoistParams* cp, const EdgeParams* es, const EncodeParams* ees, int spec_groups,
-                          hipStream_t s) {
+                          const WarmImage* warm, int* warm_wgs, hipStream_t s) {
+    if (warm_wgs) *warm_wgs = 0;
     if (sp->B <= 0 || p->st_n <= 0) return;
     const int items = (p->st_n + 3) / 4, wgs = items;
     const int gh = p->xcd_n > 0 ? (wgs + p->xcd_n - 1) / p->xcd_n * 8 : wgs;
@@ -1496,6 +1506,9 @@
         gc = (gc + (8 - p->xcd_n) - 1) / (8 - p->xcd_n) * 8;
     }
     const int pm = poll_max > 0 ? poll_max : pfsb::SB_XCHG_POLLS;
+    int gw = 0;
+    if (warm && warm->base && warm->bytes >= 16 && p->xcd_n > 0 && p->xcd_n < 8)
+        gw = 8 * pf_warm_rows(gh / 8 + (avoid > 0 ? 0 : (sp->B + 7) / 8));
     if (gc == 0 && gs == 0) {
         hipLaunchKernelGGL(k_rg_node_hs_build<HsbPlain>, dim3(gh + gb), dim3(256), 0, s, p->in_start, p->in_cnt, p->st_n0, p->st_n, p->xcd_n, gh,
                            *p, *hp, *sp, *bp, xstat, poll_sleep, avoid, pm, gb, HsbPlain{});
@@ -1505,7 +1518,9 @@
     if (gc) ex.cp = *cp;
     ex.gs = gs + pad2;
     if (gs) { ex.es = *es; ex.ees = *ees; }
-    hipLaunchKernelGGL(k_rg_node_hs_build<HsbExtra>, dim3(gh + gb + pad + gs + pad2 + gc), dim3(256), 0, s, p->in_start, p->in_cnt, p->st_n0, p->st_n,
+    ex.gw = gw;
+    if (gw) { ex.warm = *warm; if (warm_wgs) *warm_wgs = gw / 8 * p->xcd_n; }
+    hipLaunchKernelGGL(k_rg_node_hs_build<HsbExtra>, dim3(gh + gw + gb + pad + gs + pad2 + gc), dim3(256), 0, s, p->in_start, p->in_cnt, p->st_n0, p->st_n,
                        p->xcd_n, gh, *p, *hp, *sp, *bp, xstat, poll_sleep, avoid, pm, gb + pad, ex);
 }
 void pfk_pa_spec(const EdgeParams* es, const EncodeParams* ees, int groups, int after, int k, int frac, int* word, hipStream_t s) {
diff --git a/pharmacophore-diffusion_amd/engine.py b/pharmacophore-diffusion_amd/engine.py
--- a/pharmacophore-diffusion_amd/engine.py
+++ b/pharmacophore-diffusion_amd/engine.py
@@ -392,6 +392,11 @@
     def pa_check(self) -> int:
         return self.pa_check_counts()["violations"]
 
+    def l2_warm(self):
+        out = (ctypes.c_int32 * 4)()
+        self._ck(self.lib.pf_debug_l2_warm(self._h, out), "pf_debug_l2_warm")
+        return dict(zip(("merged_wgs", "merged_bytes", "fused_wgs", "fused_bytes"), list(out)))
+
     def l0_hoist(self) -> int:
         r = ctypes.c_int32()
         self._ck(self.lib.pf_debug_l0_hoist(self._h, ctypes.byref(r)), "pf_debug_l0_hoist")
```

New measurement: 678,700 sample-steps/s. -1.1%, worse.
